# danpovey/quantization

Measured on AMD Instinct MI355X. Metric: vectors encoded/sec at dim=512, 8 codebooks; uint8 codes bit-exact vs ref, higher is better.
Workload: dtype f32 (products: exact 30-bit fixed point on the i8 MFMA); 1 GPU; Quantizer.encode, dim=512, bytes_per_frame=8, codebook_size=256, refine_indexes_iters=5, batch=65536 fp32 Gaussian vectors per GPU (BASELINE.json configs[1]), seeded synthetic codebooks; global_batch=65536, parallelism=batch-sharded x1, no collective

## Files before the change

quantization_amd/csrc/mcq_api.hip:

```cpp
#include "../../include/mcq.h"
#include "mcq_kernels.h"
#include "mcq_fix_kernels.h"
#include "mcq_loss_kernels.h"
#include "mcq_tf_kernels.h"
#include "mcq_pass16_kernels.h"
#include "mcq_train_kernels.h"
#include "mcq_search_kernels.h"
#include "mcq_range_kernels.h"

#include <cstdlib>
#include <type_traits>
#include <utility>
#include <vector>

using namespace mcq;

namespace {

inline int round_up16(int d) { return (d + 15) & ~15; }
inline size_t align256(size_t v) { return (v + 255) & ~size_t(255); }
inline bool is_pow2(int v) { return v > 0 && (v & (v - 1)) == 0; }

int k_cutoff(int K, int L) {
    int kc = (K <= 16) ? 8 : 16;
    while (L >= 4) { L /= 4; kc *= 2; }
    return kc < 128 ? kc : 128;
}

struct Prepared {
    const float *C, *Q, *bias, *scales, *G, *mean, *wmu;
    const int8_t *Cf, *Wf;
    const int *Ce, *We;
};

struct PreparedLayout {
    size_t offC, offQ, offCf, offCe, offWf, offWe, offWmu, offBias, offScales, offMean, offCMean, offG, total;
};

PreparedLayout prepared_layout(int N, int K, int D) {
    const size_t nk = (size_t)N * K, Dp = round_up16(D);
    const size_t planes = fix_plane_bytes((long)nk, D), exps = (size_t)fix_round_rows((long)nk) * 4;
    PreparedLayout l;
    l.offC = 0;
    l.offQ = align256(l.offC + nk * Dp * 4);
    l.offCf = align256(l.offQ + nk * 4);
    l.offCe = align256(l.offCf + planes);
    l.offWf = align256(l.offCe + exps);
    l.offWe = align256(l.offWf + planes);
    l.offWmu = align256(l.offWe + exps);
    l.offBias = align256(l.offWmu + nk * 4);
    l.offScales = align256(l.offBias + nk * 4);
    l.offMean = align256(l.offScales + 8);
    l.offCMean = align256(l.offMean + Dp * 4);
    l.offG = align256(l.offCMean + (size_t)N * Dp * 4);
    l.total = align256(l.offG + nk * nk * 4);
    static_assert(kFixTile == 128, "");
    if (l.total < l.offBias + (nk + kFixTile) * 4) l.total = align256(l.offBias + (nk + kFixTile) * 4);
    return l;
}

Prepared prepared_view(const void *p, int N, int K, int D) {
    const PreparedLayout l = prepared_layout(N, K, D);
    const char *b = static_cast<const char *>(p);
    return Prepared{reinterpret_cast<const float *>(b + l.offC), reinterpret_cast<const float *>(b + l.offQ),
                    reinterpret_cast<const float *>(b + l.offBias), reinterpret_cast<const float *>(b + l.offScales),
                    reinterpret_cast<const float *>(b + l.offG), reinterpret_cast<const float *>(b + l.offMean),
                    reinterpret_cast<const float *>(b + l.offWmu),
                    reinterpret_cast<const int8_t *>(b + l.offCf), reinterpret_cast<const int8_t *>(b + l.offWf),
                    reinterpret_cast<const int *>(b + l.offCe), reinterpret_cast<const int *>(b + l.offWe)};
}

template <typename CT>
struct WorkspaceT {
    CT *idx, *idxB, *idxC, *final_idx;
    int *map[2], *cnt;
    float *E, *R, *xx, *XC;
    float *gterms;
    int8_t *xf;
    int *xe;
    float *tabs[2];
    TfLists tf;
};

int tf_levels(int N) { int v = 0; while ((1 << v) < N) ++v; return v; }

size_t tf_tab_floats(int N, int K) {
    const int nlev = tf_levels(N);
    size_t best = 0;
    for (int v = 2; v < nlev; ++v) {
        const size_t groups = (size_t)N >> (v + 1);
        for (int u = 1; u < v; ++u) {
            const size_t per = (size_t)1 << (v - u), kc = k_cutoff(K, 1 << u);
            const size_t f = groups * per * per * kc * kc;
            best = f > best ? f : best;
        }
    }
    return best;
}

inline size_t code_bytes_of(int K) { return K > 256 ? 2 : 1; }

size_t workspace_per_vector(int N, int K, int D) {
    const size_t cb = code_bytes_of(K);
    return 4 * cb * (size_t)N + 8 + 8 + 4 * (size_t)N + 4 * (size_t)N * K + (size_t)tf_levels(N) * N * (16 * cb + 2 * 16 + 4 * 16) + 64 +
           2 * 4 * tf_tab_floats(N, K) + 4 * (size_t)fix_round_cols(D) + 4 + 4 * (size_t)N * N;
}
size_t workspace_slack(int D) { return 48 * 256 + (size_t)kFixTile * (4 * (size_t)fix_round_cols(D) + 4); }

long default_chunk(int N, int K, int D) {
    long c = (long)(((size_t)2 << 30) / workspace_per_vector(N, K, D));
    c = c > 65536 ? 65536 : c;
    c = c < 1024 ? 1024 : c;
    return c & ~127L;
}

template <typename CT>
WorkspaceT<CT> carve(void *ws, long Bc, int N, int K, int D) {
    char *p = static_cast<char *>(ws);
    size_t off = 0;
    auto take = [&](size_t bytes) { char *q = p + off; off = align256(off + bytes); return q; };
    WorkspaceT<CT> w;
    w.idx = reinterpret_cast<CT *>(take((size_t)Bc * N * sizeof(CT)));
    w.idxB = reinterpret_cast<CT *>(take((size_t)Bc * N * sizeof(CT)));
    w.idxC = reinterpret_cast<CT *>(take((size_t)Bc * N * sizeof(CT)));
    w.final_idx = reinterpret_cast<CT *>(take((size_t)Bc * N * sizeof(CT)));
    for (int i = 0; i < 2; ++i) w.map[i] = reinterpret_cast<int *>(take((size_t)Bc * 4));
    w.cnt = reinterpret_cast<int *>(take(64 * 4));
    w.E = reinterpret_cast<float *>(take((size_t)Bc * 4));
    w.R = reinterpret_cast<float *>(take((size_t)Bc * N * 4));
    w.xx = reinterpret_cast<float *>(take((size_t)Bc * 4));
    w.gterms = reinterpret_cast<float *>(take((size_t)Bc * N * N * 4));
    w.XC = reinterpret_cast<float *>(take((size_t)Bc * N * K * 4));
    w.xf = reinterpret_cast<int8_t *>(take(fix_plane_bytes(Bc, D)));
    w.xe = reinterpret_cast<int *>(take((size_t)fix_round_rows(Bc) * 4));
    const int nlev = tf_levels(N);
    w.tf.ent = nullptr;
    w.tf.out_i64 = nullptr;
    w.tf.out_u8 = nullptr;
    w.tf.out_pack = 1;
    w.tf.map = nullptr;
    w.tf.erG = w.tf.erXC = w.tf.erxx = nullptr;
    w.tf.erE = w.tf.erR = nullptr;
    w.tf.erK = 0;
    for (int v = 0; v < kTfLevels; ++v) {
        w.tf.kc[v] = k_cutoff(K, 1 << v);
        w.tf.pos[v] = nullptr;
        w.tf.S[v] = nullptr;
        if (v >= nlev) continue;
        const int kc = w.tf.kc[v];
        if (v == 0) w.tf.ent = reinterpret_cast<uint8_t *>(take((size_t)Bc * N * kc * sizeof(CT)));
        else w.tf.pos[v] = reinterpret_cast<uint8_t *>(take((size_t)Bc * (N >> v) * kc * 2));
        w.tf.S[v] = reinterpret_cast<float *>(take((size_t)Bc * (N >> v) * kc * 4));
    }
    const size_t tf = tf_tab_floats(N, K);
    for (int i = 0; i < 2; ++i) w.tabs[i] = tf ? reinterpret_cast<float *>(take((size_t)Bc * tf * 4)) : nullptr;
    return w;
}

bool domain_ok(int N, int K, int D) {
    return is_pow2(K) && K >= 16 && K <= 1024 && is_pow2(N) && N <= 64 && (long)N * K <= 16384 && D >= 1 && D <= 16384;
}
int domain_err(int N, int K, int D = 1) {
    return (K < 16 || K > 1024 || N > 64 || (long)N * K > 16384 || D > 16384) ? MCQ_EUNSUPPORTED : MCQ_EINVAL;
}

struct Prof {
    hipStream_t stream;
    int only = -1;
    std::vector<hipEvent_t> ev;
    std::vector<int> cat, first, last;
    int open = -1;
    void begin(int category) {
        if (only >= 0 && category != only) { open = -1; return; }
        if (ev.empty() || open != (int)ev.size() - 1) {
            hipEvent_t e;
            (void)hipEventCreate(&e);
            (void)hipEventRecord(e, stream);
            ev.push_back(e);
        }
        open = (int)ev.size() - 1;
    }
    void untimed() { open = -1; }
    void end(int category) {
        if (only >= 0 && category != only) { open = -1; return; }
        hipEvent_t e;
        (void)hipEventCreate(&e);
        (void)hipEventRecord(e, stream);
        ev.push_back(e);
        first.push_back(open);
        last.push_back((int)ev.size() - 1);
        cat.push_back(category);
        open = (int)ev.size() - 1;
    }
};

thread_local int g_last_launches = 0;

#define MCQ_LAUNCH_CHECK()                               \
    do {                                                 \
        hipError_t e_ = hipGetLastError();               \
        if (e_ != hipSuccess) return (int)e_;            \
        ++g_last_launches;                               \
    } while (0)

FixRowsArgs fix_rows_args(const float *src, int xh, long R, int D, long ld, int8_t *planes, int *exps, float *xx,
                          const float *bias_src = nullptr, float *bias_dst = nullptr, const float *sub = nullptr,
                          long sub_per = 0, long sub_ld = 0, const float *dot_vec = nullptr, float *dot_out = nullptr) {
    return FixRowsArgs{src, xh, R, fix_round_rows(R), D, ld, fix_round_cols(D), planes, exps, xx, bias_src, bias_dst,
                       sub, sub_per, sub_ld, dot_vec, dot_out, nullptr};
}

int launch_fix_rows(const float *src, int xh, long R, int D, long ld, int8_t *planes, int *exps, float *xx, hipStream_t st,
                    const float *sub = nullptr, unsigned *clear = nullptr) {
    FixRowsArgs a = fix_rows_args(src, xh, R, D, ld, planes, exps, xx, nullptr, nullptr, sub, 0, 0);
    a.clear = clear;
    hipLaunchKernelGGL(k_fix_rows<4>, dim3((unsigned)(a.Rp / 4)), dim3(256), 0, st, a);
    MCQ_LAUNCH_CHECK();
    return 0;
}

int launch_fix_rows2(const FixRowsArgs &a, const FixRowsArgs &b, hipStream_t st) {
    const unsigned na = (unsigned)(a.Rp / 4), nb = (unsigned)(b.Rp / 4);
    hipLaunchKernelGGL(k_fix_rows2<4>, dim3(na + nb), dim3(256), 0, st, a, b, na);
    MCQ_LAUNCH_CHECK();
    return 0;
}

template <int MODE>
int launch_fgemm(FixGemm g, hipStream_t st) {
    static bool allowed[64] = {};
    constexpr int lds = MODE == FG_SCREEN ? kFixLdsScreen : kFixLds;
    int dev = 0;
    if (hipGetDevice(&dev) != hipSuccess || dev < 0 || dev >= 64) dev = 63;
    if (!allowed[dev] || dev == 63) {
        const hipError_t attr = hipFuncSetAttribute(reinterpret_cast<const void *>(&k_fgemm<MODE>),
                                                    hipFuncAttributeMaxDynamicSharedMemorySize, lds);
        if (attr != hipSuccess) return (int)attr;
        allowed[dev] = true;
    }
    const long MT = g.RA / kFixTile, NT = g.RB / kFixTile;
    const int H = (MODE != FG_STORE && g.K > kFixTile) ? g.K / kFixTile : 1;
    const long big = g.walk_rows ? NT : MT, small_units = (g.walk_rows ? MT : NT) / H;
    long units = (big + 7) / 8 * small_units;
    if (units > 32) units = 32;
    hipLaunchKernelGGL((k_fgemm<MODE>), dim3((unsigned)(8 * units)), dim3(512), lds, st, g);
    MCQ_LAUNCH_CHECK();
    return 0;
}

int launch_xc(const int8_t *xf, const int *xe, long B, const int8_t *Cf, const int *Ce, long nk, int D, float *out,
              hipStream_t st) {
    FixGemm g{};
    g.A = xf; g.ea = xe; g.RA = fix_round_rows(B); g.M = B;
    g.B = Cf; g.eb = Ce; g.RB = fix_round_rows(nk); g.N = nk;
    g.Dq = fix_round_cols(D);
    g.walk_rows = 0;
    g.out = out; g.ldo = nk;
    return launch_fgemm<FG_STORE>(g, st);
}

inline bool exact_logits_forced() {
    static const bool on = getenv("MCQ_EXACT_LOGITS") && atoi(getenv("MCQ_EXACT_LOGITS")) != 0;
    return on;
}

int launch_logits(const int8_t *xf, const int *xe, long B, const Prepared &P, int N, int K, int D, float lscale,
                  const float *lscale_ptr, float *logits, void *idx, hipStream_t st, unsigned *und_cnt = nullptr,
                  unsigned *und_list = nullptr) {
    const long nk = (long)N * K;
    FixGemm g{};
    g.A = P.Wf; g.ea = P.We; g.RA = fix_round_rows(nk); g.M = nk;
    g.B = xf; g.eb = xe; g.RB = fix_round_rows(B); g.N = B;
    g.Dq = fix_round_cols(D);
    g.walk_rows = 1;
    g.bias = P.bias; g.wmu = P.wmu; g.lscale = lscale; g.lscale_ptr = lscale_ptr;
    g.logits = logits; g.ldo = nk; g.idx = idx; g.idx_wide = K > 256 ? 1 : 0; g.K = K; g.ncb = N;
    if (und_cnt == nullptr) return launch_fgemm<FG_LOGITS>(g, st);
    if (logits != nullptr) return MCQ_EINVAL;
    g.und_cnt = und_cnt; g.und_list = und_list; g.und_cap = (unsigned)(B * N);
    const int rc = launch_fgemm<FG_SCREEN>(g, st);
    if (rc) return rc;
    FixRecheck r{};
    r.W = P.Wf; r.X = xf; r.ew = P.We; r.ex = xe; r.RW = g.RA; r.RX = g.RB; r.Dq = g.Dq;
    r.bias = P.bias; r.wmu = P.wmu; r.lscale_ptr = lscale_ptr; r.lscale = lscale;
    r.idx = idx; r.idx_wide = g.idx_wide; r.K = K; r.ncb = N; r.cnt = und_cnt; r.list = und_list; r.cap = g.und_cap;
    const long waves = B * N;
    hipLaunchKernelGGL(k_fscreen_recheck, dim3((unsigned)(waves < 4096 ? (waves + 3) / 4 : 1024)), dim3(256), 0, st, r);
    MCQ_LAUNCH_CHECK();
    return 0;
}

constexpr unsigned kCapStage0 = 32768, kCapWave = 65536;
inline unsigned pass_grid(unsigned full, bool capped, unsigned cap) { return (capped && full > cap) ? cap : full; }

template <int K>
int launch_tf_stage0_k(int N, const float *G, const float *XC, const tf_code_of<K> *idx, const float *R, const float *Q, long B,
                       int keep, tf_code_of<K> *ent, float *S, tf_code_of<K> *fin, const int *nact, const int *map, hipStream_t st,
                       bool capped) {
    const unsigned vgrid = (unsigned)(((B + 3) / 4) * N);
    const dim3 grid(pass_grid(vgrid, capped, kCapStage0)), block(256);
#define MCQ_S0_CASE(NN)                                                                                                            \
    case NN:                                                                                                                       \
        if (capped) hipLaunchKernelGGL((k_tf_stage0<K, NN, true>), grid, block, 0, st, G, XC, idx, R, Q, B, keep, ent, S, fin, nact, map, vgrid); \
        else hipLaunchKernelGGL((k_tf_stage0<K, NN, false>), grid, block, 0, st, G, XC, idx, R, Q, B, keep, ent, S, fin, nact, map, vgrid);      \
        break;
    switch (N) {
        MCQ_S0_CASE(1) MCQ_S0_CASE(2) MCQ_S0_CASE(4) MCQ_S0_CASE(8) MCQ_S0_CASE(16) MCQ_S0_CASE(32) MCQ_S0_CASE(64)
        default: return MCQ_EUNSUPPORTED;
    }
#undef MCQ_S0_CASE
    MCQ_LAUNCH_CHECK();
    return 0;
}

int launch_tf_stage0(int K, int N, const float *G, const float *XC, const uint16_t *idx, const float *R, const float *Q,
                     long B, int keep, uint16_t *ent, float *S, uint16_t *fin, const int *nact, const int *map, hipStream_t st,
                     bool capped) {
    switch (K) {
        case 512: return launch_tf_stage0_k<512>(N, G, XC, idx, R, Q, B, keep, ent, S, fin, nact, map, st, capped);
        case 1024: return launch_tf_stage0_k<1024>(N, G, XC, idx, R, Q, B, keep, ent, S, fin, nact, map, st, capped);
        default: return MCQ_EUNSUPPORTED;
    }
}

int launch_tf_stage0(int K, int N, const float *G, const float *XC, const uint8_t *idx, const float *R, const float *Q,
                     long B, int keep, uint8_t *ent, float *S, uint8_t *fin, const int *nact, const int *map, hipStream_t st,
                     bool capped) {
    if (K == 16 && N >= 4 && keep <= 16) {
        const dim3 grid((unsigned)((B * (N / 4) + 3) / 4)), block(256);
#define MCQ_S16_CASE(NN) \
    case NN: hipLaunchKernelGGL((k_tf_stage0_k16<NN>), grid, block, 0, st, G, XC, idx, R, Q, B, keep, ent, S, nact, map); break;
        switch (N) {
            MCQ_S16_CASE(4) MCQ_S16_CASE(8) MCQ_S16_CASE(16) MCQ_S16_CASE(32) MCQ_S16_CASE(64)
            default: return MCQ_EUNSUPPORTED;
        }
#undef MCQ_S16_CASE
        MCQ_LAUNCH_CHECK();
        return 0;
    }
    switch (K) {
        case 16: return launch_tf_stage0_k<16>(N, G, XC, idx, R, Q, B, keep, ent, S, fin, nact, map, st, capped);
        case 32: return launch_tf_stage0_k<32>(N, G, XC, idx, R, Q, B, keep, ent, S, fin, nact, map, st, capped);
        case 64: return launch_tf_stage0_k<64>(N, G, XC, idx, R, Q, B, keep, ent, S, fin, nact, map, st, capped);
        case 128: return launch_tf_stage0_k<128>(N, G, XC, idx, R, Q, B, keep, ent, S, fin, nact, map, st, capped);
        case 256: return launch_tf_stage0_k<256>(N, G, XC, idx, R, Q, B, keep, ent, S, fin, nact, map, st, capped);
        default: return MCQ_EUNSUPPORTED;
    }
}

template <typename CT>
int launch_tf_er(int N, const float *G, const float *XC, const CT *idx, const float *xx, long B, int K, float *E, float *R,
                 float *gterms, const int *nact, const int *map, hipStream_t st) {
    const dim3 grid((unsigned)((B + 3) / 4)), block(256);
    const bool direct = B <= 8192;
#define MCQ_ER_CASE(NN)                                                                                                  \
    case NN:                                                                                                             \
        if (!direct) {                                                                                                   \
            hipLaunchKernelGGL((k_tf_gram_terms<NN, CT>), dim3((unsigned)(((B + 4 * (64 / NN) - 1) / (4 * (64 / NN))) * NN)), block, 0, st, G, idx, \
                               B, K, gterms, nact);                                                                      \
            MCQ_LAUNCH_CHECK();                                                                                          \
        }                                                                                                                \
        hipLaunchKernelGGL((k_tf_er<NN, CT>), grid, block, 0, st, gterms, XC, idx, xx, B, K, E, R, nact, map,              \
                           direct ? G : static_cast<const float *>(nullptr));                                           \
        break;
    switch (N) {
        MCQ_ER_CASE(1) MCQ_ER_CASE(2) MCQ_ER_CASE(4) MCQ_ER_CASE(8) MCQ_ER_CASE(16) MCQ_ER_CASE(32) MCQ_ER_CASE(64)
        default: return MCQ_EUNSUPPORTED;
    }
#undef MCQ_ER_CASE
    MCQ_LAUNCH_CHECK();
    return 0;
}

int launch_tf_up(int kh, int kc, const TfLists &L, long B, int N, int u, int ntab, int per, const float *in, float *out,
                 const int *nact, hipStream_t st) {
    const dim3 grid((unsigned)(B * ntab)), block(64);
#define MCQ_UP_CASE(A, C) \
    if (kh == A && kc == C) { hipLaunchKernelGGL((k_tf_up<A, C>), grid, block, 0, st, L, B, N, u, ntab, per, in, out, nact); MCQ_LAUNCH_CHECK(); return 0; }
    MCQ_UP_CASE(16, 32) MCQ_UP_CASE(32, 32) MCQ_UP_CASE(32, 64) MCQ_UP_CASE(8, 16) MCQ_UP_CASE(16, 16)
#undef MCQ_UP_CASE
    return MCQ_EUNSUPPORTED;
}

template <typename CT>
int launch_tf_comb(int kh, int kc, const float *E, const TfLists &L, long B, int N, int v, int keep, const float *tabs,
                   CT *fin, const int *nact, hipStream_t st, bool capped) {
    if (fin == nullptr) capped = false;
    const dim3 grid(pass_grid((unsigned)(B * (N >> (v + 1))), capped, kCapWave)), block(64);
#define MCQ_COMB_CASE(A, C)                                                                                                        \
    if (kh == A && kc == C) {                                                                                                     \
        if (fin && capped) hipLaunchKernelGGL((k_tf_comb<A, C, true, CT, true>), grid, block, 0, st, E, L, B, N, v, keep, tabs, fin, nact); \
        else if (fin) hipLaunchKernelGGL((k_tf_comb<A, C, true, CT>), grid, block, 0, st, E, L, B, N, v, keep, tabs, fin, nact);  \
        else hipLaunchKernelGGL((k_tf_comb<A, C, false, CT>), grid, block, 0, st, E, L, B, N, v, keep, tabs, fin, nact);          \
        MCQ_LAUNCH_CHECK();                                                                                                       \
        return 0;                                                                                                                 \
    }
    MCQ_COMB_CASE(16, 32) MCQ_COMB_CASE(32, 32) MCQ_COMB_CASE(32, 64) MCQ_COMB_CASE(64, 64)
    if constexpr (sizeof(CT) == 1) { MCQ_COMB_CASE(8, 16) MCQ_COMB_CASE(16, 16) }
#undef MCQ_COMB_CASE
    return MCQ_EUNSUPPORTED;
}

enum { CAT_LOGITS = 0, CAT_XX = 1, CAT_STAGE0 = 2, CAT_XC = 3, CAT_LEVEL0 = 4, CAT_LEVEL1 = 5, CAT_TABLES = 6, CAT_COMBINE = 7,
       CAT_TABLES_UP = 8, CAT_COMBINE_UP = 9, CAT_ER = 10, CAT_LEVEL1_FUSED = 11, CAT_TAIL = 12, CAT_COUNT = 13 };
const char *const kCatNames[CAT_COUNT] = {
    "logits_product_argmax",
    "frames_to_limbs",
    "stage0_tables",
    "xc_product",
    "combine_level0",
    "combine_level1",
    "tables_level1",
    "combine_level2",
    "tables_upper_levels",
    "combine_upper_levels",
    "residual_energies",
    "level1_combines_and_tables",
    "encode_tail",
};

#define MCQ_TF_LAUNCH2(SMALLK, BIGK, grid, block, ...)                                                       \
    do {                                                                                                     \
        bool s_ = false;                                                                                     \
        if constexpr (sizeof(CT) == 1) {                                                                     \
            if (small) { hipLaunchKernelGGL(SMALLK, grid, block, 0, st, __VA_ARGS__); s_ = true; }           \
        }                                                                                                    \
        if (!s_) hipLaunchKernelGGL(BIGK, grid, block, 0, st, __VA_ARGS__);                                  \
    } while (0)
inline bool pass16_enabled() {
    static const bool on = !(getenv("MCQ_PASS16") && atoi(getenv("MCQ_PASS16")) == 0);
    return on;
}
inline long skip_min_batch() {
    const char *v = getenv("MCQ_SKIP_MIN_BATCH");
    return v ? atol(v) : 8192;
}

template <typename CT>
int run_tf_combines(const float *G, const CT *idx_cur, CT *idx_new, const WorkspaceT<CT> &w, const TfLists &L, long B, int N,
                    int K, const int *nact, hipStream_t st, Prof *prof, bool capped) {
    const bool small = (K == 16);
    const int nlev = tf_levels(N);
    {
        const int keep = (N == 2) ? 1 : L.kc[1];
        CT *fin = (N == 2) ? idx_new : nullptr;
        const dim3 grid((unsigned)(B * (N / 2)));
        if (prof) prof->begin(CAT_LEVEL0);
        bool done0 = false;
        if constexpr (sizeof(CT) == 1) {
            if (!small) {
                if (capped)
                    hipLaunchKernelGGL(k_tf_pair0s<true>, dim3(pass_grid(grid.x, true, kCapWave)), dim3(64), 0, st, G, idx_cur, w.E, L, B, N,
                                       K, keep, fin, nact);
                else
                    hipLaunchKernelGGL(k_tf_pair0s<false>, grid, dim3(64), 0, st, G, idx_cur, w.E, L, B, N, K, keep, fin, nact);
                done0 = true;
            }
        }
        if (!done0) MCQ_TF_LAUNCH2((k_tf_pair0<8, CT>), (k_tf_pair0<16, CT>), grid, dim3(64), G, idx_cur, w.E, L, B, N, K, keep, fin, nact);
        MCQ_LAUNCH_CHECK();
        if (prof) prof->end(CAT_LEVEL0);
    }
    const bool fuse_l1 = (N >= 8);
    const bool fuse_l3 = fuse_l1 && N == 16 && small;
    if (fuse_l1) {
        const int keep = L.kc[2];
        const int groups2 = N >> 3, per1 = 2, ntab1 = groups2 * per1 * per1;
        const unsigned pair_blocks = (unsigned)(B * (N / 4)), tab_blocks = (unsigned)(B * ntab1);
        const int ntab3 = fuse_l3 ? 16 : 1, per3 = fuse_l3 ? 4 : 1;
        const unsigned vgrid = pair_blocks + tab_blocks + (fuse_l3 ? (unsigned)(B * ntab3) : 0u);
        const dim3 grid(pass_grid(vgrid, capped, kCapWave));
        if (prof) prof->begin(CAT_LEVEL1_FUSED);
        if (capped)
            MCQ_TF_LAUNCH2((k_tf_level1<8, 8, CT, true>), (k_tf_level1<16, 16, CT, true>), grid, dim3(64), G, idx_cur, w.E, L, B, N, K, keep, ntab1,
                           per1, w.tabs[0], nact, pair_blocks, tab_blocks, ntab3, per3, w.tabs[1], vgrid);
        else
            MCQ_TF_LAUNCH2((k_tf_level1<8, 8, CT>), (k_tf_level1<16, 16, CT>), grid, dim3(64), G, idx_cur, w.E, L, B, N, K, keep, ntab1, per1, w.tabs[0],
                           nact, pair_blocks, tab_blocks, ntab3, per3, w.tabs[1], vgrid);
        MCQ_LAUNCH_CHECK();
        if (prof) prof->end(CAT_LEVEL1_FUSED);
    } else if (N >= 4) {
        const int keep = (N == 4) ? 1 : L.kc[2];
        CT *fin = (N == 4) ? idx_new : nullptr;
        const dim3 grid((unsigned)(B * (N / 4)));
        if (prof) prof->begin(CAT_LEVEL1);
        MCQ_TF_LAUNCH2((k_tf_pair1<8, 8, CT>), (k_tf_pair1<16, 16, CT>), grid, dim3(64), G, idx_cur, w.E, L, B, N, K, keep, fin, nact);
        MCQ_LAUNCH_CHECK();
        if (prof) prof->end(CAT_LEVEL1);
    }
    for (int v = 2; v < nlev; ++v) {
        const int groups = N >> (v + 1);
        const bool last = (v == nlev - 1);
        const int keep = last ? 1 : L.kc[v + 1];
        CT *fin = last ? idx_new : nullptr;
        const int per1 = 1 << (v - 1), ntab1 = groups * per1 * per1;
        const int cat_tab = (v == 2) ? CAT_TABLES : CAT_TABLES_UP, cat_comb = (v == 2) ? CAT_COMBINE : CAT_COMBINE_UP;
        if (!(fuse_l1 && v == 2) && !(fuse_l3 && v == 3)) {
            if (prof) prof->begin(cat_tab);
            MCQ_TF_LAUNCH2((k_tf_table1<8, 8, CT>), (k_tf_table1<16, 16, CT>), dim3((unsigned)(B * ntab1)), dim3(64), G, idx_cur, L, B, N, K, ntab1, per1,
                           w.tabs[0], nact);
            MCQ_LAUNCH_CHECK();
            if (prof) prof->end(cat_tab);
        }
        if (N == 16 && v == 3) {
            if (prof) prof->begin(cat_comb);
            const float *t3 = fuse_l3 ? w.tabs[1] : w.tabs[0];
            MCQ_TF_LAUNCH2((k_tf_comb3<8, 16, 16, CT>), (k_tf_comb3<16, 32, 32, CT>), dim3((unsigned)B), dim3(256), idx_cur, w.E, L, B, N, t3, idx_new, nact);
            MCQ_LAUNCH_CHECK();
            if (prof) prof->end(cat_comb);
            continue;
        }
        int cur = 0;
        for (int u = 2; u < v; ++u) {
            const int per = 1 << (v - u), ntab = groups * per * per;
            if (prof) prof->begin(cat_tab);
            const int rc = launch_tf_up(L.kc[u - 1], L.kc[u], L, B, N, u, ntab, per, w.tabs[cur], w.tabs[cur ^ 1], nact, st);
            if (rc) return rc;
            if (prof) prof->end(cat_tab);
            cur ^= 1;
        }
        if (prof) prof->begin(cat_comb);
        const int rc = launch_tf_comb<CT>(L.kc[v - 1], L.kc[v], w.E, L, B, N, v, keep, w.tabs[cur], fin, nact, st, capped);
        if (rc) return rc;
        if (prof) prof->end(cat_comb);
    }
    return 0;
}
#undef MCQ_TF_LAUNCH2

template <typename CT>
int run_encode_t(const float *x, long B, const void *prepared, float lscale, int N, int K, int D, int iters,
                 uint8_t *out_u8, int64_t *out_i64, void *workspace, size_t workspace_bytes, hipStream_t st,
                 Prof *prof, const int64_t *init_idx, unsigned flags, float *logits_out,
                 uint8_t *codes_also ) {
    g_last_launches = 0;
    if (!domain_ok(N, K, D)) return domain_err(N, K, D);
    if (B < 0 || iters < 0 || iters > 60 || (out_u8 == nullptr) == (out_i64 == nullptr)) return MCQ_EINVAL;
    if (sizeof(CT) > 1 && (out_u8 != nullptr || codes_also != nullptr)) return MCQ_EINVAL;
    if (B == 0) return 0;
    if (!x || !prepared || !workspace) return MCQ_EINVAL;
    const size_t per = workspace_per_vector(N, K, D), slack = workspace_slack(D);
    if (workspace_bytes < slack + per) return MCQ_EWORKSPACE;
    long chunk = (long)((workspace_bytes - slack) / per);
    if (chunk > B) chunk = B;
    if (chunk < B && chunk < 128) return MCQ_EWORKSPACE;
    if (chunk < B) chunk &= ~127L;
    const Prepared P = prepared_view(prepared, N, K, D);
    const int pack = (out_u8 != nullptr && K == 16 && N >= 2) ? 2 : 1;
    const bool want_skip = (flags & MCQ_ENCODE_ALL_PASSES) == 0 && iters >= 3;

    for (long lo = 0; lo < B; lo += chunk) {
        const long Bc = (B - lo < chunk) ? (B - lo) : chunk;
        const WorkspaceT<CT> w = carve<CT>(workspace, Bc, N, K, D);
        const int xh = (flags & MCQ_ENCODE_X_FP16) ? 1 : 0;
        const float *xc = xh ? reinterpret_cast<const float *>(reinterpret_cast<const uint16_t *>(x) + lo * D) : x + lo * D;
        int rc;
        const bool screen = init_idx == nullptr && logits_out == nullptr && (flags & MCQ_ENCODE_EXACT_LOGITS) == 0 &&
                            !exact_logits_forced() && (size_t)Bc * N < ((size_t)1 << 31);
        unsigned *const und_cnt = reinterpret_cast<unsigned *>(w.cnt + 63), *const und_list = reinterpret_cast<unsigned *>(w.XC);
        if (init_idx == nullptr || iters > 0) {
            if (prof) prof->begin(CAT_XX);
            rc = launch_fix_rows(xc, xh, Bc, D, D, w.xf, w.xe, w.xx, st, P.mean, screen ? und_cnt : nullptr);
            if (rc) return rc;
            if (prof) prof->end(CAT_XX);
        }
        if (init_idx != nullptr) {
            hipLaunchKernelGGL(k_import_indexes<CT>, dim3((unsigned)((Bc * N + 255) / 256)), dim3(256), 0, st,
                               init_idx + lo * N, Bc * N, K, w.idx);
            MCQ_LAUNCH_CHECK();
            if (prof) prof->untimed();
        } else {
            if (prof) prof->begin(CAT_LOGITS);
            rc = launch_logits(w.xf, w.xe, Bc, P, N, K, D, lscale,
                               (flags & MCQ_ENCODE_LSCALE_FROM_PREPARED) ? P.scales + 1 : nullptr,
                               logits_out ? logits_out + lo * N * K : nullptr, w.idx, st, screen ? und_cnt : nullptr, und_list);
            if (rc) return rc;
            if (prof) prof->end(CAT_LOGITS);
        }
        if (iters > 0) {
            if (prof) prof->begin(CAT_XC);
            rc = launch_xc(w.xf, w.xe, Bc, P.Cf, P.Ce, (long)N * K, D, w.XC, st);
            if (rc) return rc;
            if (prof) prof->end(CAT_XC);
        }
        const bool use_p16 = sizeof(CT) == 1 && K == 16 && (N == 16 || N == 8) && iters > 0 && prof == nullptr && pass16_enabled();
        const bool skip = want_skip && !use_p16 && Bc >= skip_min_batch();
        int iters_left = iters;
        CT *idx_cur = w.idx, *idx_new = skip ? w.idxB : w.idx, *idx_pk = w.idxC;
        const int *map_cur = nullptr, *nact = nullptr;
        int *map_nxt = w.map[0], *map_spare = w.map[1];
        float *E_cur = w.E, *R_cur = w.R, *E_alt = w.gterms, *R_alt = w.gterms + ((Bc + 3) & ~3L);
        if (skip) {
            hipLaunchKernelGGL(k_zero_counts, dim3(1), dim3(64), 0, st, w.cnt, 64);
            MCQ_LAUNCH_CHECK();
            if (prof) prof->untimed();
        }
        bool wrote_direct = false;
        if constexpr (sizeof(CT) == 1) {
            if (use_p16) {
                static bool allowed16[64] = {};
                int dev = 0;
                if (hipGetDevice(&dev) != hipSuccess || dev < 0 || dev >= 64) dev = 63;
                if (!allowed16[dev] || dev == 63) {
                    hipError_t attr = hipFuncSetAttribute(reinterpret_cast<const void *>(&k_tf_pass16<16>),
                                                          hipFuncAttributeMaxDynamicSharedMemorySize, p16_lds_bytes<16>());
                    if (attr == hipSuccess)
                        attr = hipFuncSetAttribute(reinterpret_cast<const void *>(&k_tf_pass16<8>),
                                                   hipFuncAttributeMaxDynamicSharedMemorySize, p16_lds_bytes<8>());
                    if (attr != hipSuccess) return (int)attr;
                    allowed16[dev] = true;
                }
                Pass16Args a;
                a.G = P.G; a.XC = w.XC; a.xx = w.xx; a.Q = P.Q; a.idx = w.idx; a.B = Bc; a.iters = iters;
                const bool direct_out = pack == 1;
                a.out_i64 = (direct_out && out_i64) ? out_i64 + lo * N : nullptr;
                a.out_u8 = direct_out ? (out_u8 ? out_u8 + lo * N : (codes_also ? codes_also + lo * N : nullptr)) : nullptr;
                const long wgs = (Bc + kP16Waves - 1) / kP16Waves;
                if (N == 16)
                    hipLaunchKernelGGL(k_tf_pass16<16>, dim3((unsigned)(wgs < 256 ? wgs : 256)), dim3(64 * kP16Waves), p16_lds_bytes<16>(), st, a);
                else
                    hipLaunchKernelGGL(k_tf_pass16<8>, dim3((unsigned)(wgs < 512 ? wgs : 512)), dim3(64 * kP16Waves), p16_lds_bytes<8>(), st, a);
                MCQ_LAUNCH_CHECK();
                if (direct_out) continue;
                iters_left = 0;
            }
        }
        const bool er_in_emit = (N == 4 || N == 8 || N == 16);
        bool er_ready = false;
        for (int it = 0; it < iters_left; ++it) {
            const bool last_pass = (it + 1 == iters);
            const bool capped = skip && it >= 3;
            if (!er_ready) {
                if (prof) prof->begin(CAT_ER);
                rc = launch_tf_er<CT>(N, P.G, w.XC, idx_cur, w.xx, Bc, K, E_cur, R_cur, w.gterms, nact, map_cur, st);
                if (rc) return rc;
                if (prof) prof->end(CAT_ER);
            }
            er_ready = false;
            if (prof) prof->begin(CAT_STAGE0);
            rc = launch_tf_stage0(K, N, P.G, w.XC, idx_cur, R_cur, P.Q, Bc, (N == 1) ? 1 : w.tf.kc[0], reinterpret_cast<CT *>(w.tf.ent),
                                  w.tf.S[0], (N == 1) ? idx_new : static_cast<CT *>(nullptr), nact, map_cur, st, capped);
            if (rc) return rc;
            if (prof) prof->end(CAT_STAGE0);
            bool direct_out = false;
            if (N >= 2) {
                TfLists L = w.tf;
                L.map = map_cur;
                if (er_in_emit && !last_pass) {
                    L.erG = P.G; L.erXC = w.XC; L.erxx = w.xx; L.erE = E_cur; L.erR = R_cur; L.erK = K;
                    er_ready = true;
                }
                direct_out = last_pass;
                if (direct_out) {
                    L.out_i64 = out_i64 ? out_i64 + lo * N : nullptr;
                    L.out_u8 = out_u8 ? out_u8 + lo * (N / pack) : (codes_also ? codes_also + lo * N : nullptr);
                    L.out_pack = out_u8 ? pack : 1;
                    wrote_direct = true;
                }
                WorkspaceT<CT> wc = w;
                wc.E = E_cur;
                wc.R = R_cur;
                rc = run_tf_combines<CT>(P.G, idx_cur, idx_new, wc, L, Bc, N, K, nact, st, prof, capped);
                if (rc) return rc;
            }
            if (skip && !direct_out) {
                if (prof) prof->begin(CAT_TAIL);
                hipLaunchKernelGGL(k_compact<CT>, dim3((unsigned)((Bc + 255) / 256)), dim3(256), 0, st, idx_cur, idx_new,
                                   map_cur, nact, Bc, N, last_pass ? 1 : 0, idx_pk, map_nxt, w.cnt + it,
                                   er_ready ? E_cur : nullptr, er_ready ? R_cur : nullptr, E_alt, R_alt, pack,
                                   out_u8 ? out_u8 + lo * (N / pack) : nullptr, out_i64 ? out_i64 + lo * N : nullptr,
                                   codes_also ? codes_also + lo * N : nullptr);
                MCQ_LAUNCH_CHECK();
                if (prof) prof->end(CAT_TAIL);
                CT *t = idx_cur; idx_cur = idx_pk; idx_pk = t;
                int *old_map = const_cast<int *>(map_cur);
                map_cur = map_nxt;
                map_nxt = old_map ? old_map : map_spare;
                nact = w.cnt + it;
                if (er_ready) {
                    std::swap(E_cur, E_alt);
                    std::swap(R_cur, R_alt);
                }
            }
        }
        if (wrote_direct || skip) continue;
        const long outn = (out_i64 != nullptr) ? Bc * N : Bc * (N / pack);
        if (prof) prof->begin(CAT_TAIL);
        hipLaunchKernelGGL(k_finalize<CT>, dim3((unsigned)((outn + 255) / 256)), dim3(256), 0, st, w.idx, Bc, N, pack,
                           out_u8 ? out_u8 + lo * (N / pack) : nullptr, out_i64 ? out_i64 + lo * N : nullptr,
                           codes_also ? codes_also + lo * N : nullptr);
        MCQ_LAUNCH_CHECK();
        if (prof) prof->end(CAT_TAIL);
    }
    return 0;
}

int run_encode(const float *x, long B, const void *prepared, float lscale, int N, int K, int D, int iters,
               uint8_t *out_u8, int64_t *out_i64, void *workspace, size_t workspace_bytes, hipStream_t st,
               Prof *prof, const int64_t *init_idx = nullptr, unsigned flags = 0, float *logits_out = nullptr,
               uint8_t *codes_also = nullptr) {
    if (K > 256)
        return run_encode_t<uint16_t>(x, B, prepared, lscale, N, K, D, iters, out_u8, out_i64, workspace, workspace_bytes, st, prof,
                                      init_idx, flags, logits_out, codes_also);
    return run_encode_t<uint8_t>(x, B, prepared, lscale, N, K, D, iters, out_u8, out_i64, workspace, workspace_bytes, st, prof,
                                 init_idx, flags, logits_out, codes_also);
}

int db_cw_of(int D, int K) {
    if ((D & 3) != 0) return 1;
    if (K >= 64) return 4;
    return D >= 1024 ? 4 : (D >= 512 ? 2 : 1);
}
int db_cw(const void *g, const void *out, int D, int K, long gsb, long gsn, const void *dotw = nullptr) {
    const bool al = ((D & 3) == 0) && ((gsb & 3) == 0) && ((gsn & 3) == 0) && ((reinterpret_cast<uintptr_t>(g) & 15) == 0) &&
                    ((reinterpret_cast<uintptr_t>(out) & 15) == 0) && ((reinterpret_cast<uintptr_t>(dotw) & 15) == 0);
    return al ? db_cw_of(D, K) : 1;
}
int db_chunks(int D, int cw) { return (D + 64 * cw - 1) / (64 * cw); }

template <typename IdxT>
int launch_decode_backward(const float *g, const IdxT *idx, long B, int N, int K, int D, float *out, long gsb, long gsn,
                           int idx_stride, hipStream_t st, const float *sa = nullptr, const float *sb = nullptr, float sc = 1.0f,
                           const float *dotw = nullptr, float *dot_part = nullptr) {
    const int cw = db_cw(g, out, D, K, gsb, gsn, dotw), chunks = db_chunks(D, cw);
    const long rowgroups = ((long)N * K + 3) / 4;
    long blocks;
    if (chunks <= 8 && (8 % chunks) == 0) blocks = ((rowgroups + (8 / chunks) - 1) / (8 / chunks)) * 8;
    else blocks = ((long)N * K * chunks + 3) / 4;
    const dim3 grid((unsigned)blocks), block(256);
    if (cw == 4) hipLaunchKernelGGL((k_decode_backward<IdxT, 4>), grid, block, 0, st, g, idx, B, N, K, D, chunks, out, gsb, gsn, idx_stride, sa, sb, sc, dotw, dot_part);
    else if (cw == 2) hipLaunchKernelGGL((k_decode_backward<IdxT, 2>), grid, block, 0, st, g, idx, B, N, K, D, chunks, out, gsb, gsn, idx_stride, sa, sb, sc, dotw, dot_part);
    else hipLaunchKernelGGL((k_decode_backward<IdxT, 1>), grid, block, 0, st, g, idx, B, N, K, D, chunks, out, gsb, gsn, idx_stride, sa, sb, sc, dotw, dot_part);
    hipError_t e = hipGetLastError();
    return e == hipSuccess ? 0 : (int)e;
}
}

namespace {

int search_domain(int N, int K, int D) {
    if (!domain_ok(N, K, D)) return domain_err(N, K, D);
    return K > 256 ? MCQ_EUNSUPPORTED : 0;
}

int search_check(const float *tables, long Q, const uint8_t *codes, const float *w, long B, int N, int K, int k, int metric,
                 bool outs_ok, const void *workspace) {
    if (const int rc = search_domain(N, K, 1)) return rc;
    if (k > 64) return MCQ_EUNSUPPORTED;
    if (k < 1 || Q < 0 || B < 0 || Q > 0x7fffffffL) return MCQ_EINVAL;
    if (metric != MCQ_SEARCH_L2 && metric != MCQ_SEARCH_IP && metric != MCQ_SEARCH_COS) return MCQ_EINVAL;
    if (B > 0x7fffffffL) return MCQ_EUNSUPPORTED;
    if (!outs_ok) return MCQ_EINVAL;
    if (Q == 0 || B == 0) return 0;
    if (!tables || !codes || !workspace) return MCQ_EINVAL;
    if (!w && metric != MCQ_SEARCH_IP) return MCQ_EINVAL;
    const int need = N >= 16 ? 16 : N;
    if (reinterpret_cast<uintptr_t>(codes) % need != 0) return MCQ_EINVAL;
    return 0;
}

inline int launch_rc() {
    const hipError_t e = hipGetLastError();
    return e == hipSuccess ? 0 : (int)e;
}

int allow_dynamic_lds(bool (&allowed)[64], const void *kernel, int bytes) {
    int dev = 0;
    if (hipGetDevice(&dev) != hipSuccess || dev < 0 || dev >= 64) dev = 63;
    if (!allowed[dev] || dev == 63) {
        const hipError_t attr = hipFuncSetAttribute(kernel, hipFuncAttributeMaxDynamicSharedMemorySize, bytes);
        if (attr != hipSuccess) return (int)attr;
        allowed[dev] = true;
    }
    return 0;
}

template <bool RNORM>
int code_norms(const uint8_t *codes, long B, const void *prepared, int N, int K, int D, float *out, void *stream) {
    if (const int rc = search_domain(N, K, D)) return rc;
    if (B < 0) return MCQ_EINVAL;
    if (B > 0x7fffffffL) return MCQ_EUNSUPPORTED;
    if (B == 0) return 0;
    if (!codes || !prepared || !out) return MCQ_EINVAL;
    const Prepared P = prepared_view(prepared, N, K, D);
    hipLaunchKernelGGL(k_code_norms<RNORM>, dim3((unsigned)((B + kNormWaves - 1) / kNormWaves)), dim3(64 * kNormWaves), 0,
                       static_cast<hipStream_t>(stream), codes, B, P.C, N, K, round_up16(D), out);
    return launch_rc();
}

struct TilePlan {
    int qt, qtiles, slices;
    long per_slice;
};

TilePlan tile_plan(long Q, long B, int N, int K, int waves) {
    TilePlan p;
    int cap = kScanQTMax;
    while (cap > 1 && (size_t)cap * N * K * 4 > (size_t)kScanTableLds) cap /= 2;
    int qt = 1;
    while (qt < cap && qt < Q) qt *= 2;
    p.qt = qt;
    p.qtiles = (int)((Q + qt - 1) / qt);
    long cap_slices = kScanTargetBlocks / (p.qtiles > 0 ? p.qtiles : 1);
    cap_slices = cap_slices < 1 ? 1 : (cap_slices > kScanMaxSlices ? kScanMaxSlices : cap_slices);
    const long steps = (B + 63) / 64;
    long want = (steps + waves - 1) / waves;
    want = want < 1 ? 1 : (want > cap_slices ? cap_slices : want);
    p.per_slice = (((B + want - 1) / want) + 63) / 64 * 64;
    if (p.per_slice < 64) p.per_slice = 64;
    p.slices = (int)((B + p.per_slice - 1) / p.per_slice);
    return p;
}

struct ScanPlan : TilePlan {
    size_t lds, ws_half;
};

ScanPlan scan_plan(long Q, long B, int N, int K, int k) {
    ScanPlan p{tile_plan(Q, B, N, K, kScanWaves), 0, 0};
    const size_t tab = (size_t)p.qt * N * K * 4, lists = (size_t)p.qt * kScanWaves * 64 * 8;
    p.lds = tab > lists ? tab : lists;
    p.ws_half = align256((size_t)Q * p.slices * k * 4);
    return p;
}

template <int QT, int NN, int M>
int launch_scan(const ScanPlan &p, hipStream_t st, const float *tables, int Q, const uint8_t *codes, const float *norms, long B,
                int K, int k, float *ws_s, int *ws_i) {
    static bool allowed[64] = {};
    if (const int rc = allow_dynamic_lds(allowed, reinterpret_cast<const void *>(&k_search_scan<QT, NN, M>), kScanTableLds))
        return rc;
    hipLaunchKernelGGL((k_search_scan<QT, NN, M>), dim3((unsigned)p.qtiles * (unsigned)p.slices), dim3(64 * kScanWaves), p.lds, st,
                       tables, Q, codes, norms, B, K, k, p.slices, p.per_slice, ws_s, ws_i);
    return launch_rc();
}

template <int QT, int M>
int launch_scan_n(const ScanPlan &p, hipStream_t st, const float *tables, int Q, const uint8_t *codes, const float *norms,
                  long B, int N, int K, int k, float *ws_s, int *ws_i) {
    switch (N) {
#define MCQ_SCAN_CASE(NN) \
    case NN: return launch_scan<QT, NN, M>(p, st, tables, Q, codes, norms, B, K, k, ws_s, ws_i);
        MCQ_SCAN_CASE(1) MCQ_SCAN_CASE(2) MCQ_SCAN_CASE(4) MCQ_SCAN_CASE(8) MCQ_SCAN_CASE(16) MCQ_SCAN_CASE(32) MCQ_SCAN_CASE(64)
#undef MCQ_SCAN_CASE
    }
    return MCQ_EUNSUPPORTED;
}

static_assert(kMetricL2 == MCQ_SEARCH_L2 && kMetricIP == MCQ_SEARCH_IP && kMetricCos == MCQ_SEARCH_COS, "include/mcq.h");
template <int M>
int launch_scan_qt(const ScanPlan &p, hipStream_t st, const float *tables, int Q, const uint8_t *codes, const float *w, long B,
                   int N, int K, int k, float *ws_s, int *ws_i) {
    switch (p.qt) {
        case 1: return launch_scan_n<1, M>(p, st, tables, Q, codes, w, B, N, K, k, ws_s, ws_i);
        case 2: return launch_scan_n<2, M>(p, st, tables, Q, codes, w, B, N, K, k, ws_s, ws_i);
        case 4: return launch_scan_n<4, M>(p, st, tables, Q, codes, w, B, N, K, k, ws_s, ws_i);
        case 8: return launch_scan_n<8, M>(p, st, tables, Q, codes, w, B, N, K, k, ws_s, ws_i);
        case 16: return launch_scan_n<16, M>(p, st, tables, Q, codes, w, B, N, K, k, ws_s, ws_i);
    }
    return MCQ_EUNSUPPORTED;
}

}


namespace {

struct RangePlan : TilePlan {
    size_t lds, ws_bytes;
};

RangePlan range_plan(long Q, long B, int N, int K) {
    RangePlan p{tile_plan(Q, B, N, K, kRangeWaves), 0, 0};
    p.lds = (size_t)p.qt * N * K * 4 + (size_t)kRangeWaves * p.qt * 8;
    p.ws_bytes = align256((size_t)Q * p.slices * kRangeWaves * 8);
    return p;
}

struct RangeArgs {
    const float *tables;
    int Q;
    const uint8_t *codes;
    const float *w;
    long B;
    int N, K, metric;
    const float *thr;
    int64_t *ws;
    const int64_t *lims;
    float *out_s;
    int64_t *out_i;
    long capacity;
};

template <int QT, int CH, bool FILL>
int launch_range(const RangePlan &p, hipStream_t st, const RangeArgs &a) {
    static bool allowed[64] = {};
    if (const int rc = allow_dynamic_lds(allowed, reinterpret_cast<const void *>(&k_range_sweep<QT, CH, FILL>),
                                         kScanTableLds + kRangeWaves * kScanQTMax * 8))
        return rc;
    hipLaunchKernelGGL((k_range_sweep<QT, CH, FILL>), dim3((unsigned)p.qtiles * (unsigned)p.slices), dim3(64 * kRangeWaves), p.lds,
                       st, a.tables, a.Q, a.codes, a.w, a.B, a.N, a.K, a.metric, p.slices, p.per_slice, a.thr, a.ws, a.lims,
                       a.out_s, a.out_i, a.capacity);
    return launch_rc();
}

template <int QT, bool FILL>
int launch_range_ch(const RangePlan &p, hipStream_t st, const RangeArgs &a) {
    switch (a.N < 8 ? a.N : 8) {
        case 1: return launch_range<QT, 1, FILL>(p, st, a);
        case 2: return launch_range<QT, 2, FILL>(p, st, a);
        case 4: return launch_range<QT, 4, FILL>(p, st, a);
        case 8: return launch_range<QT, 8, FILL>(p, st, a);
    }
    return MCQ_EUNSUPPORTED;
}

template <bool FILL>
int launch_range_qt(const RangePlan &p, hipStream_t st, const RangeArgs &a) {
    switch (p.qt) {
        case 1: return launch_range_ch<1, FILL>(p, st, a);
        case 2: return launch_range_ch<2, FILL>(p, st, a);
        case 4: return launch_range_ch<4, FILL>(p, st, a);
        case 8: return launch_range_ch<8, FILL>(p, st, a);
        case 16: return launch_range_ch<16, FILL>(p, st, a);
    }
    return MCQ_EUNSUPPORTED;
}

int range_check(const float *tables, long Q, const uint8_t *codes, const float *w, long B, int N, int K, int metric,
                const float *thr, const int64_t *lims, const void *workspace, size_t workspace_bytes) {
    if (const int rc = search_check(tables, Q, codes, w, B, N, K, 1, metric, lims != nullptr, workspace)) return rc;
    if (Q == 0 || B == 0) return 0;
    if (!thr) return MCQ_EINVAL;
    if (workspace_bytes < range_plan(Q, B, N, K).ws_bytes) return MCQ_EWORKSPACE;
    return 0;
}

}


extern "C" {

int mcq_abi_version(void) { return MCQ_ABI_VERSION; }

int mcq_padded_dim(int D) { return round_up16(D); }

size_t mcq_prepared_bytes(int N, int K, int D) {
    if (N <= 0 || K <= 0 || D <= 0) return 0;
    return prepared_layout(N, K, D).total;
}

static int prepare_impl(const float *centers, float cscale_exp, const float *scales_dev, const float *weight,
                        const float *bias, int N, int K, int D, void *prepared, void *stream, const float *raw_cs = nullptr,
                        const float *raw_ls = nullptr, float speed = 0.f, float *scales_out2 = nullptr) {
    if (!domain_ok(N, K, D)) return domain_err(N, K, D);
    if (!centers || !prepared || ((weight == nullptr) != (bias == nullptr))) return MCQ_EINVAL;
    hipStream_t st = static_cast<hipStream_t>(stream);
    const PreparedLayout l = prepared_layout(N, K, D);
    char *b = static_cast<char *>(prepared);
    const long rows = (long)N * K;
    const int Dp = round_up16(D);
    const unsigned grid = (unsigned)((rows + 3) / 4);
    hipLaunchKernelGGL(k_prepare_rows, dim3(grid), dim3(256), 0, st, centers, cscale_exp, 1, rows, D, Dp,
                       reinterpret_cast<float *>(b + l.offC), static_cast<float *>(nullptr) , scales_dev,
                       (scales_dev || raw_cs) ? reinterpret_cast<float *>(b + l.offScales) : static_cast<float *>(nullptr), raw_cs,
                       raw_ls, speed, scales_out2);
    hipError_t e = hipGetLastError();
    if (e != hipSuccess) return (int)e;
    if (!weight) return 0;
    const float *C = reinterpret_cast<const float *>(b + l.offC);
    float *cmean = reinterpret_cast<float *>(b + l.offCMean);
    hipLaunchKernelGGL(k_centers_mean, dim3((unsigned)(Dp / 16)), dim3(1024), 0, st, C, N, K, Dp,
                       reinterpret_cast<float *>(b + l.offMean), cmean);
    e = hipGetLastError();
    if (e != hipSuccess) return (int)e;
    int rc = launch_fix_rows2(fix_rows_args(C, 0, rows, Dp, Dp, reinterpret_cast<int8_t *>(b + l.offCf), reinterpret_cast<int *>(b + l.offCe),
                                            reinterpret_cast<float *>(b + l.offQ), nullptr, nullptr, cmean, K, Dp),
                              fix_rows_args(weight, 0, rows, D, D, reinterpret_cast<int8_t *>(b + l.offWf), reinterpret_cast<int *>(b + l.offWe),
                                            nullptr, bias, reinterpret_cast<float *>(b + l.offBias), nullptr, 0, 0,
                                            reinterpret_cast<const float *>(b + l.offMean), reinterpret_cast<float *>(b + l.offWmu)), st);
    if (rc) return rc;
    {
        rc = launch_xc(reinterpret_cast<const int8_t *>(b + l.offCf), reinterpret_cast<const int *>(b + l.offCe), rows,
                       reinterpret_cast<const int8_t *>(b + l.offCf), reinterpret_cast<const int *>(b + l.offCe), rows, D,
                       reinterpret_cast<float *>(b + l.offG), st);
        if (rc) return rc;
    }
    return 0;
}

size_t mcq_prepared_decode_bytes(int N, int K, int D) {
    if (N <= 0 || K <= 0 || D <= 0) return 0;
    return prepared_layout(N, K, D).offCf;
}

size_t mcq_prepared_mean_offset(int N, int K, int D) {
    if (N <= 0 || K <= 0 || D <= 0) return 0;
    return prepared_layout(N, K, D).offMean;
}

int mcq_prepare(const float *centers, float cscale_exp, const float *weight, const float *bias, int N, int K, int D,
                void *prepared, void *stream) {
    return prepare_impl(centers, cscale_exp, nullptr, weight, bias, N, K, D, prepared, stream);
}

int mcq_prepare_dev(const float *centers, const float *scales_exp, const float *weight, const float *bias, int N,
                    int K, int D, void *prepared, void *stream) {
    if (!scales_exp) return MCQ_EINVAL;
    return prepare_impl(centers, 1.0f, scales_exp, weight, bias, N, K, D, prepared, stream);
}

int mcq_prepare_params(const float *centers, const float *centers_scale, const float *logits_scale, float speed,
                       const float *weight, const float *bias, int N, int K, int D, void *prepared, float *scales_exp_out,
                       void *stream) {
    if (!centers_scale || !logits_scale) return MCQ_EINVAL;
    return prepare_impl(centers, 1.0f, nullptr, weight, bias, N, K, D, prepared, stream, centers_scale, logits_scale, speed,
                        scales_exp_out);
}

size_t mcq_encode_workspace_bytes(long B, int N, int K, int D) {
    if (B <= 0 || N <= 0 || K <= 0 || D <= 0 || !domain_ok(N, K, D)) return 48 * 256;
    const long dc = default_chunk(N, K, D), chunk = B < dc ? B : dc;
    return workspace_slack(D) + workspace_per_vector(N, K, D) * (size_t)chunk;
}

int mcq_encode(const float *x, long B, const void *prepared, float lscale_exp, int N, int K, int D, int refine_iters,
               uint8_t *out_u8, int64_t *out_i64, void *workspace, size_t workspace_bytes, void *stream) {
    return run_encode(x, B, prepared, lscale_exp, N, K, D, refine_iters, out_u8, out_i64, workspace,
                      workspace_bytes, static_cast<hipStream_t>(stream), nullptr);
}

int mcq_encode_ex(const float *x, long B, const void *prepared, float lscale_exp, int N, int K, int D,
                  int refine_iters, uint8_t *out_u8, int64_t *out_i64, void *workspace, size_t workspace_bytes,
                  void *stream, unsigned flags) {
    return run_encode(x, B, prepared, lscale_exp, N, K, D, refine_iters, out_u8, out_i64, workspace,
                      workspace_bytes, static_cast<hipStream_t>(stream), nullptr, nullptr, flags);
}

int mcq_refine_indexes(const float *x, long B, const void *prepared, int N, int K, int D, int refine_iters,
                       const int64_t *idx_in, int64_t *idx_out, void *workspace, size_t workspace_bytes,
                       void *stream) {
    if (B > 0 && (!idx_in || !idx_out)) return MCQ_EINVAL;
    return run_encode(x, B, prepared, 1.0f, N, K, D, refine_iters, nullptr, idx_out, workspace, workspace_bytes,
                      static_cast<hipStream_t>(stream), nullptr, B > 0 ? idx_in : nullptr);
}

int mcq_decode(const void *codes, int code_bytes, int codes_per_row, long B, const void *prepared, int N, int K, int D,
               float *out, void *stream) {
    if (!domain_ok(N, K, D)) return domain_err(N, K);
    if (B < 0 || codes_per_row <= 0 || N % codes_per_row != 0) return MCQ_EINVAL;
    const int rep = N / codes_per_row;
    if (!(rep == 1 || rep == 2 || rep == 4 || rep == 8 || rep == 16)) return MCQ_EINVAL;
    if (code_bytes != 1 && code_bytes != 8) return MCQ_EINVAL;
    if (B == 0) return 0;
    if (!codes || !prepared || !out) return MCQ_EINVAL;
    hipStream_t st = static_cast<hipStream_t>(stream);
    const Prepared P = prepared_view(prepared, N, K, D);
    const int Dp = round_up16(D);
    const unsigned grid = (unsigned)((B + 3) / 4);
    const int J = (Dp / 4 + 63) / 64;
    static const bool sliced_ok = !(getenv("MCQ_DECODE_SLICED") && atoi(getenv("MCQ_DECODE_SLICED")) == 0);
    const char *lds_env = getenv("MCQ_DECODE_LDS_MIN");
    const long lds_min_b = lds_env ? atol(lds_env) : 16384;
    {
        const char *blk_env = getenv("MCQ_DECODE_BLK");
        const int blk_mode = blk_env ? atoi(blk_env) : 1;
        const size_t lds_max = 160 * 1024, cbytes = 2 * 16384;
        int lpv = 0;
        if ((size_t)N * K * 64 + cbytes <= lds_max) lpv = 4;
        else if ((size_t)N * K * 32 + cbytes <= lds_max) lpv = 2;
        if (blk_mode != 0 && sliced_ok && rep == 1 && code_bytes == 1 && B >= lds_min_b && K >= 32 && (D & 3) == 0 && lpv != 0 &&
            (N == 4 || N == 8 || N == 16) && ((reinterpret_cast<uintptr_t>(codes) & 15) == 0) && ((reinterpret_cast<uintptr_t>(out) & 15) == 0)) {
            const int W = 4 * lpv, ns = Dp / W, per_xcd = (ns + 7) / 8;
            int groups = 256 / (8 * per_xcd);
            groups = groups < 1 ? 1 : groups;
            const unsigned g = (unsigned)(8 * per_xcd * groups);
            const long per = (((B + groups - 1) / groups) + 255) / 256 * 256;
            const size_t lds = (size_t)N * K * W * 4 + cbytes;
            const uint8_t *cp = static_cast<const uint8_t *>(codes);
#define MCQ_DECB(NN, LL)                                                                                                    \
    do {                                                                                                                    \
        static bool allowed[64] = {};                                                                                       \
        int dev = 0;                                                                                                        \
        if (hipGetDevice(&dev) != hipSuccess || dev < 0 || dev >= 64) dev = 63;                                             \
        if (!allowed[dev] || dev == 63) {                                                                                   \
            const hipError_t attr = hipFuncSetAttribute(reinterpret_cast<const void *>(&k_decode_blk<NN, LL>),              \
                                                        hipFuncAttributeMaxDynamicSharedMemorySize, (int)lds_max);          \
            if (attr != hipSuccess) return (int)attr;                                                                       \
            allowed[dev] = true;                                                                                            \
        }                                                                                                                   \
        hipLaunchKernelGGL((k_decode_blk<NN, LL>), dim3(g), dim3(1024), lds, st, cp, B, P.C, K, D, Dp, groups, per, out);   \
    } while (0)
            if (N == 4) { if (lpv == 4) MCQ_DECB(4, 4); else MCQ_DECB(4, 2); }
            else if (N == 8) { if (lpv == 4) MCQ_DECB(8, 4); else MCQ_DECB(8, 2); }
            else { if (lpv == 4) MCQ_DECB(16, 4); else MCQ_DECB(16, 2); }
#undef MCQ_DECB
            hipError_t e6 = hipGetLastError();
            return e6 == hipSuccess ? 0 : (int)e6;
        }
    }
    if (sliced_ok && rep == 1 && B >= lds_min_b && (size_t)N * K * 64 <= 144 * 1024 && K >= 32 && N >= 8) {
        const int ns = Dp / 16, per_xcd = (ns + 7) / 8;
        int groups = 256 / (8 * per_xcd);
        groups = groups < 1 ? 1 : groups;
        const unsigned g = (unsigned)(8 * per_xcd * groups);
        const size_t lds = (size_t)N * K * 64;
        if (code_bytes == 1)
            hipLaunchKernelGGL((k_decode_lds<uint8_t>), dim3(g), dim3(1024), lds, st, static_cast<const uint8_t *>(codes), B,
                               P.C, N, K, D, Dp, groups, out);
        else
            hipLaunchKernelGGL((k_decode_lds<int64_t>), dim3(g), dim3(1024), lds, st, static_cast<const int64_t *>(codes), B,
                               P.C, N, K, D, Dp, groups, out);
        hipError_t e4 = hipGetLastError();
        return e4 == hipSuccess ? 0 : (int)e4;
    }
    if (sliced_ok && rep == 1 && B >= 4096 && K >= 32) {
        int lpv = 4;
        while (lpv * 32 < Dp) lpv *= 2;
        if (lpv <= 64) {
            const int vpw = 64 / lpv;
            const unsigned g = (unsigned)(((B + 4 * vpw - 1) / (4 * vpw)) * 8);
#define MCQ_DECS_LAUNCH(T, CHH, LL)                                                                              \
    hipLaunchKernelGGL((k_decode_sliced<T, CHH, LL>), dim3(g), dim3(256), 0, st, static_cast<const T *>(codes), B, P.C, N, \
                       K, D, Dp, out)
#define MCQ_DECS_LPV(T, CHH)                                                                                     \
    switch (lpv) {                                                                                               \
        case 4: MCQ_DECS_LAUNCH(T, CHH, 4); break;                                                               \
        case 8: MCQ_DECS_LAUNCH(T, CHH, 8); break;                                                               \
        case 16: MCQ_DECS_LAUNCH(T, CHH, 16); break;                                                             \
        case 32: MCQ_DECS_LAUNCH(T, CHH, 32); break;                                                             \
        default: MCQ_DECS_LAUNCH(T, CHH, 64); break;                                                             \
    }
            if (code_bytes == 1) {
                if (N <= 4) { MCQ_DECS_LPV(uint8_t, 4) } else if (N <= 8) { MCQ_DECS_LPV(uint8_t, 8) } else { MCQ_DECS_LPV(uint8_t, 16) }
            } else {
                if (N <= 4) { MCQ_DECS_LPV(int64_t, 4) } else if (N <= 8) { MCQ_DECS_LPV(int64_t, 8) } else { MCQ_DECS_LPV(int64_t, 16) }
            }
#undef MCQ_DECS_LPV
#undef MCQ_DECS_LAUNCH
            hipError_t e3 = hipGetLastError();
            return e3 == hipSuccess ? 0 : (int)e3;
        }
    }
#define MCQ_DEC_CASE(NN, JJ)                                                                                    \
    if (code_bytes == 1 && rep == 1 && N == NN && J == JJ) {                                                    \
        hipLaunchKernelGGL((k_decode_reg<NN, JJ>), dim3(grid), dim3(256), 0, st, static_cast<const uint8_t *>(codes), \
                           B, P.C, K, D, Dp, out);                                                              \
        hipError_t e2 = hipGetLastError();                                                                      \
        return e2 == hipSuccess ? 0 : (int)e2;                                                                  \
    }
    MCQ_DEC_CASE(8, 2)
    MCQ_DEC_CASE(8, 1)
    MCQ_DEC_CASE(4, 1)
    MCQ_DEC_CASE(4, 2)
    MCQ_DEC_CASE(4, 4)
    MCQ_DEC_CASE(16, 1)
    MCQ_DEC_CASE(16, 2)
    MCQ_DEC_CASE(2, 1)
    MCQ_DEC_CASE(2, 2)
#undef MCQ_DEC_CASE
    if (code_bytes == 1)
        hipLaunchKernelGGL((k_decode<uint8_t>), dim3(grid), dim3(256), 0, st, static_cast<const uint8_t *>(codes),
                           codes_per_row, B, P.C, N, K, D, Dp, out);
    else
        hipLaunchKernelGGL((k_decode<int64_t>), dim3(grid), dim3(256), 0, st, static_cast<const int64_t *>(codes),
                           codes_per_row, B, P.C, N, K, D, Dp, out);
    hipError_t e = hipGetLastError();
    return e == hipSuccess ? 0 : (int)e;
}

int mcq_decode_backward(const float *grad_out, const int64_t *idx, long B, int N, int K, int D, float *gC,
                        void *stream) {
    if (N <= 0 || K <= 0 || D <= 0 || B < 0 || !gC) return MCQ_EINVAL;
    if (B > 0 && (!grad_out || !idx)) return MCQ_EINVAL;
    return launch_decode_backward<int64_t>(grad_out, idx, B, N, K, D, gC, (long)D, 0L, N, static_cast<hipStream_t>(stream));
}

int mcq_decode_backward_u8(const float *grad_out, const uint8_t *codes, long B, int N, int K, int D, float *gC,
                           void *stream) {
    if (K > 256) return MCQ_EUNSUPPORTED;
    if (N <= 0 || K <= 0 || D <= 0 || B < 0 || !gC) return MCQ_EINVAL;
    if (B > 0 && (!grad_out || !codes)) return MCQ_EINVAL;
    return launch_decode_backward<uint8_t>(grad_out, codes, B, N, K, D, gC, (long)D, 0L, N, static_cast<hipStream_t>(stream));
}

int mcq_scatter_rows(const float *grad, long stride_b, long stride_n, const int64_t *idx, int idx_stride, long B, int N,
                     int K, int D, float *out, void *stream) {
    if (N <= 0 || K <= 0 || D <= 0 || B < 0 || !out || idx_stride < N) return MCQ_EINVAL;
    if (B > 0 && (!grad || !idx)) return MCQ_EINVAL;
    return launch_decode_backward<int64_t>(grad, idx, B, N, K, D, out, stride_b, stride_n, idx_stride, static_cast<hipStream_t>(stream));
}

int mcq_jcl_prefix_fwd(const float *hp, const float *emb, const int64_t *idx, long B, int N, int K, int H, float scale,
                       float *A, void *stream) {
    if (N < 2 || K < 1 || H < 1 || B < 0) return MCQ_EINVAL;
    if (B == 0) return 0;
    if (!hp || !emb || !idx || !A) return MCQ_EINVAL;
    hipLaunchKernelGGL(k_jcl_prefix_fwd, dim3((unsigned)((B + 3) / 4)), dim3(256), 0, static_cast<hipStream_t>(stream), hp,
                       emb, idx, B, N, K, H, scale, A);
    hipError_t e = hipGetLastError();
    return e == hipSuccess ? 0 : (int)e;
}

int mcq_jcl_prefix_bwd(const float *A, const float *gA, long B, int N, int H, float scale, float *g_hp, float *gE,
                       void *stream) {
    if (N < 2 || H < 1 || B < 0) return MCQ_EINVAL;
    if (B == 0) return 0;
    if (!A || !gA || !g_hp || !gE) return MCQ_EINVAL;
    hipLaunchKernelGGL(k_jcl_prefix_bwd, dim3((unsigned)((B + 3) / 4)), dim3(256), 0, static_cast<hipStream_t>(stream), A,
                       gA, B, N, H, scale, g_hp, gE);
    hipError_t e = hipGetLastError();
    return e == hipSuccess ? 0 : (int)e;
}

namespace {
struct LogitsWs {
    uint8_t *idx8;
    int8_t *xf;
    int *xe;
    size_t total;
};
LogitsWs logits_ws(void *ws, long B, int N, int D) {
    char *p = static_cast<char *>(ws);
    LogitsWs w;
    size_t off = 0;
    w.idx8 = reinterpret_cast<uint8_t *>(p + off);
    off = align256(off + (size_t)B * N);
    w.xf = reinterpret_cast<int8_t *>(p + off);
    off = align256(off + fix_plane_bytes(B, D));
    w.xe = reinterpret_cast<int *>(p + off);
    off = align256(off + (size_t)fix_round_rows(B) * 4);
    w.total = off;
    return w;
}
}

size_t mcq_logits_workspace_bytes(long B, int N, int D) {
    if (B <= 0 || N <= 0 || D <= 0) return 256;
    return logits_ws(nullptr, B, N, D).total;
}

int mcq_logits(const float *x, long B, const void *prepared, float lscale_exp, int N, int K, int D, float *out,
               void *workspace, size_t workspace_bytes, void *stream) {
    if (!domain_ok(N, K, D)) return MCQ_EUNSUPPORTED;
    if (B == 0) return 0;
    if (!x || !prepared || !out || B < 0 || !workspace) return MCQ_EINVAL;
    if (workspace_bytes < mcq_logits_workspace_bytes(B, N, D)) return MCQ_EWORKSPACE;
    hipStream_t st = static_cast<hipStream_t>(stream);
    const Prepared P = prepared_view(prepared, N, K, D);
    const LogitsWs w = logits_ws(workspace, B, N, D);
    int rc = launch_fix_rows(x, 0, B, D, D, w.xf, w.xe, nullptr, st, P.mean);
    if (rc) return rc;
    return launch_logits(w.xf, w.xe, B, P, N, K, D, lscale_exp, nullptr, out, nullptr, st);
}

int mcq_logits_argmax(const float *x, long B, const void *prepared, float lscale_exp, int N, int K, int D,
                      float *logits_out, int64_t *argmax_out, void *workspace, size_t workspace_bytes, void *stream,
                      unsigned flags) {
    if (!domain_ok(N, K, D) || K > 256) return MCQ_EUNSUPPORTED;
    if (B < 0) return MCQ_EINVAL;
    if (B == 0) return 0;
    if (!x || !prepared || !logits_out || !argmax_out || !workspace) return MCQ_EINVAL;
    if (workspace_bytes < mcq_logits_workspace_bytes(B, N, D)) return MCQ_EWORKSPACE;
    hipStream_t st = static_cast<hipStream_t>(stream);
    const Prepared P = prepared_view(prepared, N, K, D);
    const LogitsWs w = logits_ws(workspace, B, N, D);
    int rc = launch_fix_rows(x, (flags & MCQ_ENCODE_X_FP16) ? 1 : 0, B, D, D, w.xf, w.xe, nullptr, st, P.mean);
    if (rc) return rc;
    rc = launch_logits(w.xf, w.xe, B, P, N, K, D, lscale_exp,
                       (flags & MCQ_ENCODE_LSCALE_FROM_PREPARED) ? P.scales + 1 : nullptr, logits_out, w.idx8, st);
    if (rc) return rc;
    hipLaunchKernelGGL(k_export_indexes, dim3((unsigned)((B * N + 255) / 256)), dim3(256), 0, st, w.idx8, B * N, argmax_out);
    MCQ_LAUNCH_CHECK();
    return 0;
}

int mcq_logits_refine(const float *x, long B, const void *prepared, float lscale_exp, int N, int K, int D, int refine_iters,
                      float *logits_out, int64_t *idx_out, void *workspace, size_t workspace_bytes, void *stream,
                      unsigned flags) {
    return mcq_logits_refine_codes(x, B, prepared, lscale_exp, N, K, D, refine_iters, logits_out, idx_out, nullptr, workspace,
                                   workspace_bytes, stream, flags);
}

int mcq_logits_refine_codes(const float *x, long B, const void *prepared, float lscale_exp, int N, int K, int D, int refine_iters,
                            float *logits_out, int64_t *idx_out, uint8_t *codes_out, void *workspace, size_t workspace_bytes,
                            void *stream, unsigned flags) {
    if (K > 256) return MCQ_EUNSUPPORTED;
    if (B > 0 && (!logits_out || !idx_out)) return MCQ_EINVAL;
    return run_encode(x, B, prepared, lscale_exp, N, K, D, refine_iters, nullptr, idx_out, workspace, workspace_bytes,
                      static_cast<hipStream_t>(stream), nullptr, nullptr, flags | MCQ_ENCODE_ALL_PASSES, logits_out,
                      codes_out);
}

namespace {
long loss_rows_per_chunk(long B) {
    long r = (B + 1023) / 1024;
    r = r < 64 ? 64 : r;
    return (r + 15) / 16 * 16;
}
long loss_chunks(long B) { const long r = loss_rows_per_chunk(B); return (B + r - 1) / r; }
}

size_t mcq_loss_workspace_bytes(long B, int N, int K) {
    if (B <= 0) return 256;
    return (size_t)loss_chunks(B) * N * (2 * (size_t)K + 1) * sizeof(float) + 256;
}

int mcq_loss_fwd(const float *logits, const int64_t *idx, long B, int N, int K, float *lse, float *chosen_sum,
                 float *prob_sum, float *count, void *workspace, size_t workspace_bytes, void *stream) {
    if (!is_pow2(K) || K < 16 || K > 256 || N < 1) return MCQ_EUNSUPPORTED;
    if (B <= 0) return MCQ_EINVAL;
    if (!logits || !idx || !lse || !chosen_sum || !prob_sum || !count || !workspace) return MCQ_EINVAL;
    if (workspace_bytes < mcq_loss_workspace_bytes(B, N, K)) return MCQ_EWORKSPACE;
    hipStream_t st = static_cast<hipStream_t>(stream);
    const long rpc = loss_rows_per_chunk(B), chunks = loss_chunks(B);
    float *pp = static_cast<float *>(workspace);
    float *pc = pp + chunks * N * K;
    float *ph = pc + chunks * N * K;
    const dim3 grid((unsigned)(chunks * N)), block(64 * kLossWaves);
#define MCQ_LOSS_CASE(KK)                                                                                             \
    case KK: hipLaunchKernelGGL((k_loss_fwd<KK>), grid, block, 0, st, logits, idx, B, N, rpc, lse, pp, pc, ph); break;
    switch (K) {
        MCQ_LOSS_CASE(16) MCQ_LOSS_CASE(32) MCQ_LOSS_CASE(64) MCQ_LOSS_CASE(128) MCQ_LOSS_CASE(256)
        default: return MCQ_EUNSUPPORTED;
    }
#undef MCQ_LOSS_CASE
    MCQ_LAUNCH_CHECK();
    hipLaunchKernelGGL(k_loss_reduce, dim3((unsigned)N), dim3(256), 0, st, pp, pc, ph, chunks, N, K, prob_sum, count,
                       chosen_sum);
    MCQ_LAUNCH_CHECK();
    return 0;
}

int mcq_loss_bwd(const float *logits, const int64_t *idx, const float *lse, long B, int N, int K, const float *g_chosen,
                 const float *g_prob, float *grad_logits, void *stream) {
    if (!is_pow2(K) || K < 16 || K > 256 || N < 1) return MCQ_EUNSUPPORTED;
    if (B <= 0) return MCQ_EINVAL;
    if (!logits || !idx || !lse || !g_chosen || !g_prob || !grad_logits) return MCQ_EINVAL;
    hipStream_t st = static_cast<hipStream_t>(stream);
    const int rpw = K < 64 ? 64 / K : 1;
    const long rows = B * N;
    const dim3 grid((unsigned)((rows + (long)kLossWaves * rpw - 1) / ((long)kLossWaves * rpw))), block(64 * kLossWaves);
#define MCQ_LOSS_CASE(KK)                                                                                             \
    case KK: hipLaunchKernelGGL((k_loss_bwd<KK>), grid, block, 0, st, logits, idx, lse, B, N, g_chosen, g_prob, grad_logits); break;
    switch (K) {
        MCQ_LOSS_CASE(16) MCQ_LOSS_CASE(32) MCQ_LOSS_CASE(64) MCQ_LOSS_CASE(128) MCQ_LOSS_CASE(256)
        default: return MCQ_EUNSUPPORTED;
    }
#undef MCQ_LOSS_CASE
    MCQ_LAUNCH_CHECK();
    return 0;
}

int mcq_loss_tail(const float *sums, const float *prob_sum, const float *count, int N, int K, float entropy_scale,
                  float *losses, float *g, float *g_prob, void *stream) {
    if (!is_pow2(K) || K < 16 || K > 256 || N < 1 || N > 64) return MCQ_EUNSUPPORTED;
    if (!sums || !prob_sum || !count || !losses || !g || !g_prob) return MCQ_EINVAL;
    hipLaunchKernelGGL(k_loss_tail, dim3(1), dim3(256), 0, static_cast<hipStream_t>(stream), sums, prob_sum, count, N, K,
                       entropy_scale, losses, g, g_prob);
    MCQ_LAUNCH_CHECK();
    return 0;
}

int mcq_recon_fwd(const float *x, const int64_t *idx, long B, const void *prepared, const float *mean, int N, int K,
                  int D, float *err, float *num_part, float *den_part, void *stream) {
    if (!domain_ok(N, K, D) || K > 256) return MCQ_EUNSUPPORTED;
    if (B <= 0) return MCQ_EINVAL;
    if (!x || !idx || !prepared || !mean || !err || !num_part || !den_part) return MCQ_EINVAL;
    const Prepared P = prepared_view(prepared, N, K, D);
    hipLaunchKernelGGL(k_recon_fwd, dim3((unsigned)((B + 3) / 4)), dim3(256), 0, static_cast<hipStream_t>(stream), x, idx, B,
                       P.C, mean, N, K, D, round_up16(D), err, num_part, den_part);
    MCQ_LAUNCH_CHECK();
    return 0;
}


namespace {
bool wgrad_use_bf3(long B, int M, int D) {
    static const bool f32_only = getenv("MCQ_WGRAD_F32") && atoi(getenv("MCQ_WGRAD_F32")) != 0;
    return !f32_only && (M % kWbM) == 0 && (D % kWbN) == 0 && M >= 1024 && B >= 2048;
}
int wgrad_splits_bf3(long B, int M, int D) {
    const long tiles = (long)(M / kWbM) * (D / kWbN);
    long s = (256 + tiles / 2) / tiles;
    const long max_s = B / 512;
    s = s > max_s ? max_s : s;
    return (int)(s < 1 ? 1 : s);
}

int wgrad_splits(long B, int M, int D) {
    const long tiles = (long)((M + kWgM - 1) / kWgM) * ((D + kWgN - 1) / kWgN);
    long s = 2048 / tiles;
    const long max_s = (B + 127) / 128;
    s = s > max_s ? max_s : s;
    return (int)(s < 1 ? 1 : (s > 64 ? 64 : s));
}
}

size_t mcq_weight_grad_workspace_bytes(long B, int M, int D) {
    if (B <= 0 || M <= 0 || D <= 0) return 256;
    return (size_t)wgrad_splits(B, M, D) * ((size_t)M * D + M) * sizeof(float) + 256;
}

int mcq_weight_grad(const float *G, const float *x, long B, int M, int D, const float *scale_dev, float *gW, float *gb,
                    void *workspace, size_t workspace_bytes, void *stream) {
    if (B <= 0 || M <= 0 || D <= 0 || (M & 15) != 0) return MCQ_EINVAL;
    if (!G || !x || !scale_dev || !gW || !gb || !workspace) return MCQ_EINVAL;
    if (workspace_bytes < mcq_weight_grad_workspace_bytes(B, M, D)) return MCQ_EWORKSPACE;
    hipStream_t st = static_cast<hipStream_t>(stream);
    const bool bf3 = wgrad_use_bf3(B, M, D);
    const int splits = bf3 ? wgrad_splits_bf3(B, M, D) : wgrad_splits(B, M, D);
    long rps = (B + splits - 1) / splits;
    rps = (rps + 31) / 32 * 32;
    float *part = static_cast<float *>(workspace);
    float *partb = part + (size_t)splits * M * D;
    if (bf3) {
        hipLaunchKernelGGL(k_wgrad_bf3, dim3((unsigned)((M / kWbM) * (D / kWbN) * splits)), dim3(512), 0, st, G, x, B, M, D, rps, part, partb);
    } else {
        const unsigned grid = (unsigned)(((M + kWgM - 1) / kWgM) * ((D + kWgN - 1) / kWgN) * splits);
        hipLaunchKernelGGL((k_wgrad_tn<16>), dim3(grid), dim3(256), 0, st, G, x, B, M, D, rps, part, partb);
    }
    MCQ_LAUNCH_CHECK();
    const long MN = (long)M * D;
    hipLaunchKernelGGL(k_wgrad_reduce, dim3((unsigned)((MN / 4 + 255) / 256)), dim3(256), 0, st, part, partb, splits, MN, M,
                       scale_dev, gW, gb);
    MCQ_LAUNCH_CHECK();
    return 0;
}

int mcq_adam_step(float *p, const float *g, float *m, float *v, long n, double lr, double beta1, double beta2, double eps,
                  double weight_decay, double bias_correction1, double bias_correction2_sqrt, void *stream) {
    if (n < 0 || (n > 0 && (!p || !g || !m || !v))) return MCQ_EINVAL;
    if (n == 0) return 0;
    long blocks = (n / 4 + 255) / 256;
    blocks = blocks < 1 ? 1 : (blocks > 2048 ? 2048 : blocks);
    hipLaunchKernelGGL(k_adam, dim3((unsigned)blocks), dim3(256), 0, static_cast<hipStream_t>(stream), p, g, m, v, n,
                       (float)(lr / bias_correction1), (float)(1.0 - beta1), (float)beta2, (float)(1.0 - beta2), (float)eps,
                       (float)weight_decay, (float)bias_correction2_sqrt);
    MCQ_LAUNCH_CHECK();
    return 0;
}

int mcq_loss_head_tail(const float *num_part, const float *den_part, long nparts, const float *chosen_n, int N, float batch,
                       float *head, const float *prob_sum, const float *count, int K, float entropy_scale, float *losses,
                       float *g, float *g_prob, void *stream) {
    if (!is_pow2(K) || K < 16 || K > 256 || N < 1 || N > 64) return MCQ_EUNSUPPORTED;
    if (nparts <= 0 || !num_part || !den_part || !chosen_n || !head || !prob_sum || !count || !losses || !g || !g_prob) return MCQ_EINVAL;
    hipLaunchKernelGGL(k_loss_head_tail, dim3(1), dim3(256), 0, static_cast<hipStream_t>(stream), num_part, den_part, nparts,
                       chosen_n, N, batch, head, prob_sum, count, K, entropy_scale, losses, g, g_prob);
    MCQ_LAUNCH_CHECK();
    return 0;
}
int mcq_loss_head(const float *num_part, const float *den_part, long nparts, const float *chosen_n, int N, float batch,
                  float *head, void *stream) {
    if (nparts <= 0 || N <= 0 || !num_part || !den_part || !chosen_n || !head) return MCQ_EINVAL;
    hipLaunchKernelGGL(k_loss_head, dim3(1), dim3(256), 0, static_cast<hipStream_t>(stream), num_part, den_part, nparts, chosen_n,
                       N, batch, head);
    MCQ_LAUNCH_CHECK();
    return 0;
}

int mcq_scales_exp(const float *centers_scale, const float *logits_scale, float speed, float *out2, void *stream) {
    if (!centers_scale || !logits_scale || !out2) return MCQ_EINVAL;
    hipLaunchKernelGGL(k_scales, dim3(1), dim3(64), 0, static_cast<hipStream_t>(stream), centers_scale, logits_scale, speed, out2);
    MCQ_LAUNCH_CHECK();
    return 0;
}

long mcq_decode_backward_waves(int N, int K, int D) { return (long)N * K * db_chunks(D, db_cw_of(D, K)); }

int mcq_decode_backward_u8_ex(const float *grad_out, const uint8_t *codes, long B, int N, int K, int D, float *gC,
                              const float *sa, const float *sb, float sc, const float *dotw, float *dot_part, void *stream) {
    if (K > 256) return MCQ_EUNSUPPORTED;
    if (N <= 0 || K <= 0 || D <= 0 || B < 0 || !gC) return MCQ_EINVAL;
    if (B > 0 && (!grad_out || !codes)) return MCQ_EINVAL;
    if ((dotw == nullptr) != (dot_part == nullptr)) return MCQ_EINVAL;
    if ((D & 3) == 0 && db_cw(grad_out, gC, D, K, D, 0, dotw) != db_cw_of(D, K)) return MCQ_EINVAL;
    const int rc = launch_decode_backward<uint8_t>(grad_out, codes, B, N, K, D, gC, (long)D, 0L, N, static_cast<hipStream_t>(stream),
                                                   sa, sb, sc, dotw, dot_part);
    if (rc) return rc;
    ++g_last_launches;
    return 0;
}

long mcq_loss_bwd_waves(long B, int N, int K) {
    const int rpw = K < 64 ? 64 / K : 1;
    const long rows = B * N;
    return ((rows + (long)kLossWaves * rpw - 1) / ((long)kLossWaves * rpw)) * kLossWaves;
}

int mcq_loss_bwd_ex(const float *logits, const int64_t *idx, const float *lse, long B, int N, int K, const float *g_chosen,
                    const float *g_prob, float *grad_logits, const float *bias, float *dot_part, void *stream) {
    if (!is_pow2(K) || K < 16 || K > 256 || N < 1) return MCQ_EUNSUPPORTED;
    if (B <= 0) return MCQ_EINVAL;
    if (!logits || !idx || !lse || !g_chosen || !g_prob || !grad_logits || !bias || !dot_part) return MCQ_EINVAL;
    hipStream_t st = static_cast<hipStream_t>(stream);
    const int rpw = K < 64 ? 64 / K : 1;
    const long rows = B * N;
    const dim3 grid((unsigned)((rows + (long)kLossWaves * rpw - 1) / ((long)kLossWaves * rpw))), block(64 * kLossWaves);
#define MCQ_LOSS_CASE(KK)                                                                                             \
    case KK: hipLaunchKernelGGL((k_loss_bwd<KK>), grid, block, 0, st, logits, idx, lse, B, N, g_chosen, g_prob, grad_logits, bias, dot_part); break;
    switch (K) {
        MCQ_LOSS_CASE(16) MCQ_LOSS_CASE(32) MCQ_LOSS_CASE(64) MCQ_LOSS_CASE(128) MCQ_LOSS_CASE(256)
        default: return MCQ_EUNSUPPORTED;
    }
#undef MCQ_LOSS_CASE
    MCQ_LAUNCH_CHECK();
    return 0;
}

int mcq_grad_tail(const float *part_c, long n_c, const float *sa, const float *sb, float sc, const float *part_l, long n_l,
                  float speed, float *out_c, float *out_l, void *stream) {
    if (n_c < 0 || n_l < 0 || (n_c > 0 && !part_c) || (n_l > 0 && !part_l)) return MCQ_EINVAL;
    hipLaunchKernelGGL(k_grad_tail, dim3(1), dim3(1024), 0, static_cast<hipStream_t>(stream), part_c, n_c, sa, sb, sc, part_l, n_l,
                       speed, out_c, out_l);
    MCQ_LAUNCH_CHECK();
    return 0;
}

int mcq_search_tables(const void *q, int q_is_fp16, long Q, const void *prepared, int N, int K, int D, float *tables_out,
                      void *stream) {
    if (const int rc = search_domain(N, K, D)) return rc;
    if (Q < 0 || Q > 0x7fffffffL) return MCQ_EINVAL;
    if (Q == 0) return 0;
    if (!q || !prepared || !tables_out) return MCQ_EINVAL;
    const Prepared P = prepared_view(prepared, N, K, D);
    const int NK = N * K;
    hipLaunchKernelGGL(k_search_tables, dim3((unsigned)((Q + kTabQueries - 1) / kTabQueries), (unsigned)((NK + kTabRows - 1) / kTabRows)),
                       dim3(256), 0, static_cast<hipStream_t>(stream), q, q_is_fp16 ? 1 : 0, (int)Q, P.C, NK, D, round_up16(D),
                       tables_out);
    return launch_rc();
}

int mcq_code_norms(const uint8_t *codes, long B, const void *prepared, int N, int K, int D, float *norms_out, void *stream) {
    return code_norms<false>(codes, B, prepared, N, K, D, norms_out, stream);
}

size_t mcq_search_workspace_bytes(long Q, long B, int N, int K, int k) {
    if (Q <= 0 || B <= 0 || k < 1 || k > 64 || B > 0x7fffffffL || Q > 0x7fffffffL || search_domain(N, K, 1) != 0) return 256;
    return 2 * scan_plan(Q, B, N, K, k).ws_half;
}

int mcq_code_rnorms(const uint8_t *codes, long B, const void *prepared, int N, int K, int D, float *rnorms_out, void *stream) {
    return code_norms<true>(codes, B, prepared, N, K, D, rnorms_out, stream);
}

int mcq_rnorms_from_norms(const float *norms, long B, float *rnorms_out, void *stream) {
    if (B < 0) return MCQ_EINVAL;
    if (B > 0x7fffffffL) return MCQ_EUNSUPPORTED;
    if (B == 0) return 0;
    if (!norms || !rnorms_out) return MCQ_EINVAL;
    hipLaunchKernelGGL(k_rnorms_from_norms, dim3((unsigned)((B + 255) / 256)), dim3(256), 0, static_cast<hipStream_t>(stream),
                       norms, B, rnorms_out);
    return launch_rc();
}

int mcq_search_scan(const float *tables, long Q, const uint8_t *codes, const float *norms, long B, int N, int K, int k,
                    float *out_score, int64_t *out_index, void *workspace, size_t workspace_bytes, void *stream) {
    return mcq_search_scan_metric(tables, Q, codes, norms, B, N, K, k, MCQ_SEARCH_L2, out_score, out_index, workspace,
                                  workspace_bytes, stream);
}

int mcq_search_scan_metric(const float *tables, long Q, const uint8_t *codes, const float *w, long B, int N, int K, int k,
                           int metric, float *out_score, int64_t *out_index, void *workspace, size_t workspace_bytes,
                           void *stream) {
    if (const int rc = search_check(tables, Q, codes, w, B, N, K, k, metric, Q == 0 || (out_score && out_index), workspace))
        return rc;
    if (Q == 0) return 0;
    hipStream_t st = static_cast<hipStream_t>(stream);
    ScanPlan p{};
    float *ws_s = nullptr;
    int *ws_i = nullptr;
    if (B > 0) {
        p = scan_plan(Q, B, N, K, k);
        if (workspace_bytes < 2 * p.ws_half) return MCQ_EWORKSPACE;
        ws_s = static_cast<float *>(workspace);
        ws_i = reinterpret_cast<int *>(static_cast<char *>(workspace) + p.ws_half);
        int rc = MCQ_EUNSUPPORTED;
        switch (metric) {
            case MCQ_SEARCH_L2: rc = launch_scan_qt<kMetricL2>(p, st, tables, (int)Q, codes, w, B, N, K, k, ws_s, ws_i); break;
            case MCQ_SEARCH_IP: rc = launch_scan_qt<kMetricIP>(p, st, tables, (int)Q, codes, nullptr, B, N, K, k, ws_s, ws_i); break;
            case MCQ_SEARCH_COS: rc = launch_scan_qt<kMetricCos>(p, st, tables, (int)Q, codes, w, B, N, K, k, ws_s, ws_i); break;
        }
        if (rc != 0) return rc;
    }
    hipLaunchKernelGGL(k_search_merge, dim3((unsigned)Q), dim3(64), 0, st, ws_s, ws_i, p.slices, k, out_score, out_index);
    return launch_rc();
}

size_t mcq_search_range_workspace_bytes(long Q, long B, int N, int K) {
    if (Q <= 0 || B <= 0 || B > 0x7fffffffL || Q > 0x7fffffffL || search_domain(N, K, 1) != 0) return 256;
    return range_plan(Q, B, N, K).ws_bytes;
}

int mcq_search_range_count(const float *tables, long Q, const uint8_t *codes, const float *w, long B, int N, int K, int metric,
                           const float *thr, int64_t *lims, void *workspace, size_t workspace_bytes, void *stream) {
    if (const int rc = range_check(tables, Q, codes, w, B, N, K, metric, thr, lims, workspace, workspace_bytes)) return rc;
    hipStream_t st = static_cast<hipStream_t>(stream);
    const bool empty = Q == 0 || B == 0;
    if (!empty) {
        const RangePlan p = range_plan(Q, B, N, K);
        int64_t *ws = static_cast<int64_t *>(workspace);
        const RangeArgs a{tables, (int)Q, codes, metric == MCQ_SEARCH_IP ? nullptr : w, B, N, K, metric, thr, ws, nullptr,
                          nullptr, nullptr, 0};
        if (const int rc = launch_range_qt<false>(p, st, a)) return rc;
        hipLaunchKernelGGL(k_range_offsets, dim3((unsigned)Q), dim3(64), 0, st, ws, p.slices * kRangeWaves, lims);
        if (const int rc = launch_rc()) return rc;
    }
    hipLaunchKernelGGL(k_range_lims, dim3(1), dim3(64), 0, st, lims, Q, empty ? 1 : 0);
    return launch_rc();
}

int mcq_search_range_fill(const float *tables, long Q, const uint8_t *codes, const float *w, long B, int N, int K, int metric,
                          const float *thr, const int64_t *lims, float *out_score, int64_t *out_index, long capacity,
                          void *workspace, size_t workspace_bytes, void *stream) {
    if (const int rc = range_check(tables, Q, codes, w, B, N, K, metric, thr, lims, workspace, workspace_bytes)) return rc;
    if (capacity < 0) return MCQ_EINVAL;
    if (Q == 0 || B == 0 || capacity == 0) return 0;
    if (!out_score || !out_index) return MCQ_EINVAL;
    const RangePlan p = range_plan(Q, B, N, K);
    const RangeArgs a{tables, (int)Q, codes, metric == MCQ_SEARCH_IP ? nullptr : w, B, N, K, metric, thr,
                      static_cast<int64_t *>(workspace), lims, out_score, out_index, capacity};
    return launch_range_qt<true>(p, static_cast<hipStream_t>(stream), a);
}

int mcq_last_encode_launches(void) { return g_last_launches; }

int mcq_test_select(const float *scores, int cases, int per_lane, int cnt, float *out_v, int *out_p, void *stream) {
    if (!scores || !out_v || !out_p || cases <= 0 || cnt < 1 || cnt > 64) return MCQ_EINVAL;
    hipStream_t st = static_cast<hipStream_t>(stream);
    switch (per_lane) {
        case 1: hipLaunchKernelGGL((k_test_select<1>), dim3(cases), dim3(64), 0, st, scores, cnt, out_v, out_p); break;
        case 4: hipLaunchKernelGGL((k_test_select<4>), dim3(cases), dim3(64), 0, st, scores, cnt, out_v, out_p); break;
        case 16: hipLaunchKernelGGL((k_test_select<16>), dim3(cases), dim3(64), 0, st, scores, cnt, out_v, out_p); break;
        case -4: hipLaunchKernelGGL((k_test_select<4, kSlotMajor>), dim3(cases), dim3(64), 0, st, scores, cnt, out_v, out_p); break;
        case -16: hipLaunchKernelGGL((k_test_select<16, kSlotMajor>), dim3(cases), dim3(64), 0, st, scores, cnt, out_v, out_p); break;
        case -1004: hipLaunchKernelGGL((k_test_select<4, kAnyOrder>), dim3(cases), dim3(64), 0, st, scores, cnt, out_v, out_p); break;
        default: return MCQ_EINVAL;
    }
    hipError_t e = hipGetLastError();
    return e == hipSuccess ? 0 : (int)e;
}

#ifdef MCQ_STAMPS
int mcq_debug_stamps(unsigned long long *host_dst, long count, int clear) {
    const long total = (long)kStampKernels * kStampWaves * kStampSlots;
    if (count > total) count = total;
    if (hipDeviceSynchronize() != hipSuccess) return MCQ_EINVAL;
    if (host_dst && count > 0 &&
        hipMemcpyFromSymbol(host_dst, HIP_SYMBOL(g_stamps), (size_t)count * 8, 0, hipMemcpyDeviceToHost) != hipSuccess) return MCQ_EINVAL;
    if (clear) {
        void *p = nullptr;
        if (hipGetSymbolAddress(&p, HIP_SYMBOL(g_stamps)) != hipSuccess || hipMemset(p, 0, (size_t)total * 8) != hipSuccess) return MCQ_EINVAL;
    }
    return (int)kStampSlots;
}
#endif

const char *mcq_profile_category_name(int category) {
    return (category >= 0 && category < CAT_COUNT) ? kCatNames[category] : nullptr;
}

int mcq_profile_encode(const float *x, long B, const void *prepared, float lscale_exp, int N, int K, int D,
                       int refine_iters, void *workspace, size_t workspace_bytes, void *stream, float *ms_out,
                       int *launches_out, int cap) {
    hipStream_t st = static_cast<hipStream_t>(stream);
    const bool wide = K > 256;
    const size_t need = (size_t)B * N * (wide ? 8 : 1);
    uint8_t *dummy = nullptr;
    if (!ms_out || cap <= 0) return MCQ_EINVAL;
    const hipError_t me = hipMalloc(reinterpret_cast<void **>(&dummy), need ? need : 1);
    if (me != hipSuccess) return (int)me;
    for (int i = 0; i < cap; ++i) { ms_out[i] = 0.f; if (launches_out) launches_out[i] = 0; }
    int rc = 0;
    for (int only = 0; only < CAT_COUNT && rc == 0; ++only) {
        Prof prof;
        prof.stream = st;
        prof.only = only;
        rc = run_encode(x, B, prepared, lscale_exp, N, K, D, refine_iters, wide ? nullptr : dummy,
                        wide ? reinterpret_cast<int64_t *>(dummy) : nullptr, workspace, workspace_bytes, st, &prof, nullptr,
                        MCQ_ENCODE_ALL_PASSES);
        (void)hipStreamSynchronize(st);
        for (size_t i = 0; rc == 0 && i < prof.cat.size(); ++i) {
            float ms = 0.f;
            (void)hipEventElapsedTime(&ms, prof.ev[prof.first[i]], prof.ev[prof.last[i]]);
            if (prof.cat[i] < cap) { ms_out[prof.cat[i]] += ms; if (launches_out) launches_out[prof.cat[i]] += 1; }
        }
        for (hipEvent_t e : prof.ev) (void)hipEventDestroy(e);
    }
    (void)hipFree(dummy);
    return rc == 0 ? CAT_COUNT : rc;
}

}
```

quantization_amd/csrc/mcq_tf_kernels.h:

```cpp
#pragma once
#include "mcq_kernels.h"

#include <type_traits>

namespace mcq {

constexpr int kTfLevels = 6;

template <int K>
using tf_code_of = std::conditional_t<(K > 256), uint16_t, uint8_t>;

struct TfLists {
    uint8_t *ent;
    uint8_t *pos[kTfLevels];
    float *S[kTfLevels];
    int kc[kTfLevels];
    int64_t *out_i64;
    uint8_t *out_u8;
    int out_pack;
    const int *map;
    const float *erG, *erXC, *erxx;
    float *erE, *erR;
    int erK;
};

__device__ __forceinline__ float shfl_f(float v, int src) {
    return __int_as_float(__builtin_amdgcn_ds_bpermute(src << 2, __float_as_int(v)));
}

#ifdef MCQ_STAMPS
constexpr int kStampSlots = 8, kStampWaves = 1 << 14, kStampKernels = 4;
__device__ unsigned long long g_stamps[kStampKernels * kStampWaves * kStampSlots];
struct Stamps {
    unsigned long long t[kStampSlots];
    __device__ __forceinline__ Stamps() { for (int i = 0; i < kStampSlots; ++i) t[i] = 0; t[0] = __builtin_amdgcn_s_memtime(); }
    __device__ __forceinline__ void at(int k) { asm volatile("s_waitcnt vmcnt(0) lgkmcnt(0)" ::: "memory"); t[k] = __builtin_amdgcn_s_memtime(); }
    __device__ __forceinline__ void flush(int kernel, unsigned wg, int every) {
        if (wg % (unsigned)every != 0 || (threadIdx.x & 63) != 0 || (threadIdx.x >> 6) != 0) return;
        const unsigned slot = (wg / (unsigned)every) & (kStampWaves - 1);
        unsigned long long *d = g_stamps + ((size_t)kernel * kStampWaves + slot) * kStampSlots;
        t[kStampSlots - 1] = __builtin_amdgcn_s_memtime();
        for (int i = 0; i < kStampSlots; ++i) d[i] = t[i];
    }
};
#else
struct Stamps {
    __device__ __forceinline__ void at(int) {}
    __device__ __forceinline__ void flush(int, unsigned, int) {}
};
#endif


template <int N, typename CT = uint8_t>
__global__ void __launch_bounds__(256)
k_tf_gram_terms(const float *__restrict__ G, const CT *__restrict__ idx, long B, int K, float *__restrict__ gterms,
                const int *__restrict__ nact) {
    constexpr int VW = 64 / N;
    if (nact) B = *nact;
    const int m = (int)(blockIdx.x % N);
    const long b = ((long)(blockIdx.x / N) * 4 + (threadIdx.x >> 6)) * VW + lane_id() / N;
    const int m2 = lane_id() % N;
    if (b >= B) return;
    const CT *id = idx + b * N;
    const int NK = N * K;
    gterms[(b * N + m) * N + m2] = G[((size_t)(m * K + id[m]) << __builtin_ctz((unsigned)NK)) + m2 * K + id[m2]];
}

template <int N, bool FROM_REG, typename CT = uint8_t>
__device__ __forceinline__ void tf_er_wave(long b, long bx, const CT *__restrict__ id, int e_reg,
                                           const float *__restrict__ gterms, const float *__restrict__ Gdirect,
                                           const float *__restrict__ XC, const float *__restrict__ xx, int K,
                                           float *__restrict__ E_out, float *__restrict__ R_out) {
    constexpr int NT = (N * N + 63) / 64;
    const int lane = lane_id();
    const int NK = N * K;
#define MCQ_ER_CODE(m) (FROM_REG ? __builtin_amdgcn_ds_bpermute((m) << 2, e_reg) : (int)id[FROM_REG ? 0 : (m)])
    float gt[NT];
#pragma unroll
    for (int j = 0; j < NT; ++j) {
        const int t = lane + 64 * j;
        const int tc = t < N * N ? t : 0;
        const float g = Gdirect ? Gdirect[(size_t)((tc / N) * K + MCQ_ER_CODE(tc / N)) * NK + (tc % N) * K + MCQ_ER_CODE(tc % N)]
                                : gterms[b * (N * N) + tc];
        gt[j] = t < N * N ? g : 0.f;
    }
    const int lm = lane < N ? lane : 0;
    const int clm = MCQ_ER_CODE(lm);
#undef MCQ_ER_CODE
    const float xt = lane < N ? XC[(size_t)bx * NK + lm * K + clm] : 0.f;
    const float xxb = xx[bx];
    float gp = gt[0];
#pragma unroll
    for (int j = 1; j < NT; ++j) gp = gp + gt[j];
    const float gsum = wave_sum_butterfly(gp), xsum = wave_sum_butterfly(xt);
    const float E = (gsum - 2.0f * xsum) + xxb;
    const int n = lane < N ? lane : 0;
    float col = 0.f, gnn = 0.f;
#pragma unroll
    for (int m = 0; m < N; ++m) {
        const float v = shfl_f(gt[(m * N) / 64], (m * N + n) & 63);
        col = (m == 0) ? v : col + v;
        if (m == n) gnn = v;
    }
    const float xo = col - xt;
    const float Rv = (E - 2.0f * xo) + gnn;
    if (lane < N) R_out[b * N + lane] = Rv;
    if (lane == 0) E_out[b] = E;
}

template <int N, typename CT = uint8_t>
__global__ void __launch_bounds__(256)
k_tf_er(const float *__restrict__ gterms, const float *__restrict__ XC, const CT *__restrict__ idx,
        const float *__restrict__ xx, long B, int K, float *__restrict__ E_out, float *__restrict__ R_out,
        const int *__restrict__ nact, const int *__restrict__ map, const float *__restrict__ Gdirect) {
    if (nact) B = *nact;
    const long b = (long)blockIdx.x * 4 + (threadIdx.x >> 6);
    if (b >= B) return;
    const long bx = map ? (long)map[b] : b;
    tf_er_wave<N, false, CT>(b, bx, idx + b * N, 0, gterms, Gdirect, XC, xx, K, E_out, R_out);
}

template <int K, int N>
__device__ __forceinline__ void
tf_stage0_body(unsigned bid, unsigned vgrid, const float *__restrict__ G, const float *__restrict__ XC, const tf_code_of<K> *__restrict__ idx,
               const float *__restrict__ R, const float *__restrict__ Q, long B, int keep,
               tf_code_of<K> *__restrict__ ent_out, float *__restrict__ S_out, tf_code_of<K> *__restrict__ idx_final ,
               const int *__restrict__ nact, const int *__restrict__ map) {
    using CT = tf_code_of<K>;
    constexpr int CB = (int)sizeof(CT);
    constexpr int VPL = (K >= 64) ? K / 64 : 1;
    constexpr int NK = N * K;
    constexpr int CH = (N - 1 < 8) ? (N > 1 ? N - 1 : 1) : 8;
    __shared__ u64 sel[4][kSelectLdsU64];
    Stamps stp;
    if (nact) B = *nact;
    int n;
    long b;
    if constexpr (N > 8) {
        const unsigned per_phase = vgrid / (N / 8);
        const unsigned ph = bid / per_phase, r = bid - ph * per_phase;
        n = (int)(r & 7u) + 8 * (int)ph;
        b = (long)(r >> 3) * 4 + (threadIdx.x >> 6);
    } else {
        n = bid & (N - 1);
        b = (long)(bid / N) * 4 + (threadIdx.x >> 6);
    }
    if (b >= B) return;
    const int lane = lane_id();
    const bool act = VPL * lane < K;
    const int k0 = act ? VPL * lane : 0;
    const CT *id = idx + b * N;
    const float *xc = XC + ((size_t)(map ? (long)map[b] : b) * NK + n * K + k0);
    const float *q = Q + n * K + k0;
    float xcv[VPL], qv[VPL];
    if constexpr (VPL == 4) {
        const f32x4 x4 = __builtin_nontemporal_load(reinterpret_cast<const f32x4 *>(xc)), q4 = *reinterpret_cast<const f32x4 *>(q);
#pragma unroll
        for (int i = 0; i < 4; ++i) { xcv[i] = x4[i]; qv[i] = q4[i]; }
    } else if constexpr (VPL % 4 == 0) {
#pragma unroll
        for (int i4 = 0; i4 < VPL / 4; ++i4) {
            const f32x4 x4 = reinterpret_cast<const f32x4 *>(xc)[i4], q4 = reinterpret_cast<const f32x4 *>(q)[i4];
#pragma unroll
            for (int i = 0; i < 4; ++i) { xcv[4 * i4 + i] = x4[i]; qv[4 * i4 + i] = q4[i]; }
        }
    } else {
#pragma unroll
        for (int i = 0; i < VPL; ++i) { xcv[i] = xc[i]; qv[i] = q[i]; }
    }
    const float Rv = R[(long)__builtin_amdgcn_readfirstlane((int)b) * N + n];
    __builtin_amdgcn_sched_barrier(0);
    unsigned long long iw[N * CB >= 8 ? N * CB / 8 : 1];
    if constexpr (N * CB >= 8) {
        const unsigned long long *ip =
            reinterpret_cast<const unsigned long long *>(idx) + (size_t)__builtin_amdgcn_readfirstlane((int)b) * (N * CB / 8);
#pragma unroll
        for (int q8 = 0; q8 < N * CB / 8; ++q8) iw[q8] = ip[q8];
    }
    auto code = [&](int m) -> int {
        if constexpr (N * CB >= 8) return (int)((iw[(m * CB) >> 3] >> (8 * ((m * CB) & 7))) & (CB == 1 ? 0xffull : 0xffffull));
        else return (int)id[m];
    };
    float t[VPL];
#pragma unroll
    for (int i = 0; i < VPL; ++i) t[i] = 0.f;
#pragma unroll
    for (int j0 = 0; j0 < N - 1; j0 += CH) {
        float gv[CH][VPL];
#pragma unroll
        for (int u = 0; u < CH; ++u) {
            const int j = j0 + u < N - 1 ? j0 + u : N - 2;
            const int m = j < n ? j : j + 1;
            const float *p = G + ((size_t)(m * K + code(m)) * NK + n * K + k0);
            if constexpr (VPL % 4 == 0) {
#pragma unroll
                for (int i4 = 0; i4 < VPL / 4; ++i4) {
                    const f32x4 t4 = reinterpret_cast<const f32x4 *>(p)[i4];
#pragma unroll
                    for (int i = 0; i < 4; ++i) gv[u][4 * i4 + i] = t4[i];
                }
            } else {
#pragma unroll
                for (int i = 0; i < VPL; ++i) gv[u][i] = p[i];
            }
        }
#pragma unroll
        for (int u = 0; u < CH; ++u)
            if (j0 + u < N - 1) {
#pragma unroll
                for (int i = 0; i < VPL; ++i) t[i] = (j0 + u == 0) ? gv[u][i] : t[i] + gv[u][i];
            }
    }
    float sv[VPL];
    int sp[VPL];
#pragma unroll
    for (int i = 0; i < VPL; ++i) {
        const float X = t[i] - xcv[i];
        sv[i] = act ? (Rv + qv[i]) + 2.0f * X : INFINITY;
        sp[i] = act ? k0 + i : kBigPos;
    }
    stp.at(1);
    float ov;
    int op, dst;
    bool has;
    wave_select_set<VPL>(sv, sp, keep, K, sel[threadIdx.x >> 6], has, dst, ov, op);
    stp.at(2);
    stp.flush(0, bid, 16);
    if (N == 1) {
        if (lane == 0) idx_final[b] = (CT)op;
        return;
    }
    if (has) {
        ent_out[(b * N + n) * keep + dst] = (CT)op;
        S_out[(b * N + n) * keep + dst] = ov;
    }
}

template <int K, int N, bool STRIDED = false>
__global__ void __launch_bounds__(256)
k_tf_stage0(const float *__restrict__ G, const float *__restrict__ XC, const tf_code_of<K> *__restrict__ idx,
            const float *__restrict__ R, const float *__restrict__ Q, long B, int keep,
            tf_code_of<K> *__restrict__ ent_out, float *__restrict__ S_out, tf_code_of<K> *__restrict__ idx_final ,
            const int *__restrict__ nact, const int *__restrict__ map, unsigned vgrid) {
    if constexpr (!STRIDED) {
        tf_stage0_body<K, N>(blockIdx.x, gridDim.x, G, XC, idx, R, Q, B, keep, ent_out, S_out, idx_final, nact, map);
        return;
    }
    const unsigned per = (N > 8) ? vgrid / (N / 8) : vgrid;
    const unsigned nr = nact ? (unsigned)((*nact + 3) / 4) * (N > 8 ? 8u : (unsigned)N) : per;
    const unsigned need = (N > 8) ? nr * (N / 8) : nr;
    for (unsigned c = blockIdx.x; c < need; c += gridDim.x) {
        const unsigned vb = (N > 8) ? (c / nr) * per + c % nr : c;
        tf_stage0_body<K, N>(vb, vgrid, G, XC, idx, R, Q, B, keep, ent_out, S_out, idx_final, nact, map);
        wave_lds_fence();
    }
}

template <int N>
__global__ void __launch_bounds__(256)
k_tf_stage0_k16(const float *__restrict__ G, const float *__restrict__ XC, const uint8_t *__restrict__ idx,
                const float *__restrict__ R, const float *__restrict__ Q, long B, int keep,
                uint8_t *__restrict__ ent_out, float *__restrict__ S_out, const int *__restrict__ nact,
                const int *__restrict__ map) {
    static_assert(N >= 4, "");
    constexpr int K = 16, NK = N * K, NG = N / 4;
    if (nact) B = *nact;
    const long w = (long)blockIdx.x * 4 + (threadIdx.x >> 6);
    const long b = w / NG;
    const int n0 = 4 * (int)(w % NG);
    if (b >= B) return;
    const int lane = lane_id();
    const int n = n0 + (lane >> 4), k = lane & 15;
    const float xcv = XC[(size_t)(map ? (long)map[b] : b) * NK + n0 * K + lane];
    const float qv = Q[n0 * K + lane];
    const float Rv = R[b * N + n];
    const long bu = __builtin_amdgcn_readfirstlane((int)b);
    unsigned long long iw[N >= 8 ? N / 8 : 1];
    if constexpr (N >= 8) {
        const unsigned long long *ip = reinterpret_cast<const unsigned long long *>(idx) + (size_t)bu * (N / 8);
#pragma unroll
        for (int q8 = 0; q8 < N / 8; ++q8) iw[q8] = ip[q8];
    } else {
        iw[0] = (unsigned long long)reinterpret_cast<const uint32_t *>(idx)[bu];
    }
    auto code = [&](int m) -> int { return (int)((iw[m >> 3] >> (8 * (m & 7))) & 0xffull) & (K - 1); };
    constexpr int CH = N < 8 ? N : 8;
    float t = 0.f;
    bool started = false;
#pragma unroll
    for (int m0 = 0; m0 < N; m0 += CH) {
        float gv[CH];
#pragma unroll
        for (int u = 0; u < CH; ++u) gv[u] = G[(size_t)((m0 + u) * K + code(m0 + u)) * NK + n0 * K + lane];
#pragma unroll
        for (int u = 0; u < CH; ++u) {
            const bool use = (m0 + u) != n;
            const float sum = t + gv[u];
            t = use ? (started ? sum : gv[u]) : t;
            started = started || use;
        }
    }
    const float X = t - xcv;
    const float sv = (Rv + qv) + 2.0f * X;
    const uint32_t hi = ord32(sv), lo = (uint32_t)k;
    const u64 key = ((u64)hi << 32) | lo;
    int rnk = 0;
#define MCQ_ROR(r)                                                                                                      \
    {                                                                                                                   \
        const u64 o = ((u64)(uint32_t)dpp_i<0x120 + r>((int)hi) << 32) | (uint32_t)dpp_i<0x120 + r>((int)lo);           \
        rnk += (o < key) ? 1 : 0;                                                                                       \
    }
    MCQ_ROR(1) MCQ_ROR(2) MCQ_ROR(3) MCQ_ROR(4) MCQ_ROR(5) MCQ_ROR(6) MCQ_ROR(7) MCQ_ROR(8)
    MCQ_ROR(9) MCQ_ROR(10) MCQ_ROR(11) MCQ_ROR(12) MCQ_ROR(13) MCQ_ROR(14) MCQ_ROR(15)
#undef MCQ_ROR
    const bool take = rnk < keep;
    const u64 tm = __ballot(take);
    const uint32_t rowbits = (uint32_t)(tm >> (lane & 48)) & 0xffffu;
    const int dst = __popc(rowbits & ((1u << k) - 1u));
    if (take) {
        ent_out[(b * N + n) * keep + dst] = (uint8_t)k;
        S_out[(b * N + n) * keep + dst] = sv;
    }
}

template <int KC, typename CT = uint8_t>
__device__ __forceinline__ void tf_leaf(const float *__restrict__ G, int NK, int K, int n, int m,
                                        const CT *__restrict__ en, const CT *__restrict__ em, int old_n,
                                        int old_m, float (&d)[KC * KC / 64]) {
    constexpr int VPL = KC * KC / 64;
    const int lane = lane_id();
    const int i = (VPL * lane) / KC, j0 = (VPL * lane) % KC;
    const uint32_t rown = (uint32_t)(n * K), colm = (uint32_t)(m * K);
    const int nksh = __builtin_ctz((unsigned)NK);
    const int bl = lane < 2 * KC ? lane : 2 * KC;
    const CT *bp = bl < KC ? en + bl : em + (bl < 2 * KC ? bl - KC : 0);
    int e_i = en[i], e_b = *bp;
    uint32_t w4 = 0;
    int ej[VPL];
    constexpr bool kPacked = (VPL == 4 && sizeof(CT) == 1);
    if constexpr (kPacked) {
        w4 = *reinterpret_cast<const uint32_t *>(em + j0);
        asm volatile("" : "+v"(e_i), "+v"(e_b), "+v"(w4));
    } else {
#pragma unroll
        for (int v = 0; v < VPL; ++v) ej[v] = em[j0 + v];
        asm volatile("" : "+v"(e_i), "+v"(e_b), "+v"(ej[0]));
    }
    const uint32_t si = rown + (uint32_t)e_i;
    const uint32_t br = bl < KC ? rown + (uint32_t)e_b : rown + (uint32_t)old_n;
    const uint32_t bc = (bl >= KC && bl < 2 * KC) ? colm + (uint32_t)e_b : colm + (uint32_t)old_m;
    float g[VPL];
    if constexpr (kPacked) {
#pragma unroll
        for (int v = 0; v < 4; ++v) g[v] = G[(si << nksh) + colm + ((w4 >> (8 * v)) & 0xffu)];
    } else {
#pragma unroll
        for (int v = 0; v < VPL; ++v) g[v] = G[(si << nksh) + colm + (uint32_t)ej[v]];
    }
    const float bv = G[(br << nksh) + bc];
    const float u = shfl_f(bv, i), w = shfl_f(bv, 2 * KC);
#pragma unroll
    for (int v = 0; v < VPL; ++v) {
        const float vj = shfl_f(bv, KC + j0 + v);
        d[v] = ((g[v] - u) - vj) + w;
    }
}

__device__ __attribute__((noinline)) void tf_er_next(const float *G, const float *XC, const float *xx, int K, float *E, float *R,
                                                     long b, long bx, int N, int e) {
    if (N == 8) tf_er_wave<8, true, uint8_t>(b, bx, nullptr, e, nullptr, G, XC, xx, K, E, R);
    else if (N == 4) tf_er_wave<4, true, uint8_t>(b, bx, nullptr, e, nullptr, G, XC, xx, K, E, R);
    else if (N == 16) tf_er_wave<16, true, uint8_t>(b, bx, nullptr, e, nullptr, G, XC, xx, K, E, R);
}

template <typename CT>
__device__ __forceinline__ void tf_emit(const TfLists &L, long b, int N, int nlev, int win, CT *__restrict__ idx_out) {
    const int n = lane_id();
    int e = 0;
    if (n < N) {
        int v = nlev - 1;
        int g = n >> v;
        int p = (g & 1) ? win % L.kc[v] : win / L.kc[v];
        while (v > 0) {
            const int child = (n >> (v - 1)) & 1;
            p = L.pos[v][((b * (N >> v) + g) * L.kc[v] + p) * 2 + child];
            --v;
            g = n >> v;
        }
        e = reinterpret_cast<const CT *>(L.ent)[(b * N + n) * L.kc[0] + p];
        idx_out[b * N + n] = (CT)e;
    }
    const long row = (L.map && (L.out_i64 || L.out_u8 || L.erE)) ? (long)L.map[b] : b;
    if (L.out_i64 && n < N) L.out_i64[row * N + n] = e;
    if (L.out_u8) {
        if (L.out_pack == 2) {
            const int hi = __builtin_amdgcn_ds_bpermute(((n + 1) & 63) << 2, e);
            if (n < N && (n & 1) == 0) L.out_u8[row * (N / 2) + n / 2] = (uint8_t)(e + 16 * hi);
        } else if (n < N) {
            L.out_u8[row * N + n] = (uint8_t)e;
        }
    }
    if (L.erE) tf_er_next(L.erG, L.erXC, L.erxx, L.erK, L.erE, L.erR, b, row, N, e);
}

template <int VPL, typename CT = uint8_t, int LAYOUT = kLaneMajor>
__device__ __forceinline__ void tf_finish(const float (&sv)[VPL], const int (&sp)[VPL], int keep, int KCin, u64 *scratch,
                                          const TfLists &L, int vout , long b, int N,
                                          int gout, CT *__restrict__ idx_final) {
    if (idx_final != nullptr) {
        float bv = INFINITY;
        int bp = kBigPos;
#pragma unroll
        for (int i = 0; i < VPL; ++i) lexmin(bv, bp, sv[i], sp[i]);
        wave_lexmin(bv, bp);
        int win = __builtin_amdgcn_readfirstlane(bp);
        if (win > KCin * KCin - 1) win = KCin * KCin - 1;
        tf_emit(L, b, N, vout, win, idx_final);
        return;
    }
    float ov;
    int op, dst;
    bool has;
    wave_select_set<VPL, LAYOUT>(sv, sp, keep, KCin * KCin, scratch, has, dst, ov, op);
    if (has) {
        const long o = (b * (N >> vout) + gout) * keep + dst;
        L.pos[vout][2 * o] = (uint8_t)(op / KCin);
        L.pos[vout][2 * o + 1] = (uint8_t)(op % KCin);
        L.S[vout][o] = ov;
    }
}

template <int KC, typename CT = uint8_t>
__global__ void __launch_bounds__(64)
k_tf_pair0(const float *__restrict__ G, const CT *__restrict__ idx, const float *__restrict__ E, TfLists L, long B,
           int N, int K, int keep, CT *__restrict__ idx_final, const int *__restrict__ nact) {
    constexpr int VPL = KC * KC / 64;
    __shared__ u64 scratch[kSelectLdsU64];
    Stamps stp;
    if (nact) B = *nact;
    const int Gout = N >> 1;
    const int g = (int)(blockIdx.x & (unsigned)(Gout - 1));
    const long b = (long)(blockIdx.x >> __builtin_ctz((unsigned)Gout));
    if (b >= B) return;
    const int lane = lane_id();
    const int n = 2 * g, m = n + 1;
    const CT *en = reinterpret_cast<const CT *>(L.ent) + (b * N + n) * KC, *em = reinterpret_cast<const CT *>(L.ent) + (b * N + m) * KC;
    const int i = (VPL * lane) / KC, j0 = (VPL * lane) % KC;
    const float Eb = E[b];
    const float se = L.S[0][(b * N + n) * KC + i];
    float so[VPL];
#pragma unroll
    for (int v = 0; v < VPL; ++v) so[v] = L.S[0][(b * N + m) * KC + j0 + v];
    float d[VPL];
    stp.at(1);
    tf_leaf<KC, CT>(G, N * K, K, n, m, en, em, idx[b * N + n], idx[b * N + m], d);
    float sv[VPL];
    int sp[VPL];
#pragma unroll
    for (int v = 0; v < VPL; ++v) {
        sv[v] = ((se + so[v]) - Eb) + 2.0f * d[v];
        sp[v] = VPL * lane + v;
    }
    stp.at(2);
    tf_finish<VPL, CT>(sv, sp, keep, KC, scratch, L, 1, b, N, g, idx_final);
    stp.at(3);
    stp.flush(1, blockIdx.x, 64);
}

__device__ __forceinline__ void
tf_pair0s_body(unsigned bid, const float *__restrict__ G, const uint8_t *__restrict__ idx, const float *__restrict__ E, const TfLists &L,
               long B, int N, int K, int keep, uint8_t *__restrict__ idx_final, const int *__restrict__ nact) {
    constexpr int KC = 16, VPL = 4;
    __shared__ u64 scratch[kSelectLdsU64];
    Stamps stp;
    if (nact) B = *nact;
    const int Gout = N >> 1;
    const int g = (int)(bid & (unsigned)(Gout - 1));
    const long b = (long)(bid >> __builtin_ctz((unsigned)Gout));
    if (b >= B) return;
    const int lane = lane_id();
    const int n = 2 * g, m = n + 1;
    const int q4 = lane >> 4, c = lane & 15;
    const uint8_t *en = L.ent + (b * N + n) * KC, *em = en + KC;
    const float *Sn = L.S[0] + (b * N + n) * KC, *Sm = Sn + KC;
    const uint32_t *enw = reinterpret_cast<const uint32_t *>(en);
    uint32_t rw[VPL];
#pragma unroll
    for (int v = 0; v < VPL; ++v) rw[v] = enw[v];
    int e_j = em[c];
    int e_b = en[c];
    int old_n = idx[b * N + n], old_m = idx[b * N + m];
    const float sn_c = Sn[c], so = Sm[c];
    const float Eb = E[b];
    asm volatile("" : "+v"(e_j), "+v"(e_b), "+v"(old_n), "+v"(old_m));
    stp.at(1);
    const int nksh = __builtin_ctz((unsigned)(N * K));
    const uint32_t rown = (uint32_t)(n * K), colm = (uint32_t)(m * K);
    float gq[VPL];
#pragma unroll
    for (int v = 0; v < VPL; ++v) {
        const uint32_t e_i = (rw[v] >> (8 * q4)) & 0xffu;
        gq[v] = G[((rown + e_i) << nksh) + colm + (uint32_t)e_j];
    }
    const uint32_t br = lane < KC ? rown + (uint32_t)e_b : rown + (uint32_t)old_n;
    const uint32_t bc = (lane >= KC && lane < 2 * KC) ? colm + (uint32_t)e_j : colm + (uint32_t)old_m;
    const float bv = G[(br << nksh) + bc];
    const float vj = shfl_f(bv, KC + c), w = shfl_f(bv, 2 * KC);
    float sv[VPL];
    int sp[VPL];
#pragma unroll
    for (int v = 0; v < VPL; ++v) {
        const int i = 4 * v + q4;
        const float u = shfl_f(bv, i), se = shfl_f(sn_c, i);
        const float d = ((gq[v] - u) - vj) + w;
        sv[v] = ((se + so) - Eb) + 2.0f * d;
        sp[v] = 64 * v + lane;
    }
    stp.at(2);
    tf_finish<VPL, uint8_t, kSlotMajor>(sv, sp, keep, KC, scratch, L, 1, b, N, g, idx_final);
    stp.at(3);
    stp.flush(1, bid, 64);
}

template <bool STRIDED = false>
__global__ void __launch_bounds__(64)
k_tf_pair0s(const float *__restrict__ G, const uint8_t *__restrict__ idx, const float *__restrict__ E, TfLists L, long B,
            int N, int K, int keep, uint8_t *__restrict__ idx_final, const int *__restrict__ nact) {
    if constexpr (!STRIDED) {
        tf_pair0s_body(blockIdx.x, G, idx, E, L, B, N, K, keep, idx_final, nact);
        return;
    }
    const unsigned need = nact ? (unsigned)*nact * (unsigned)(N >> 1) : gridDim.x;
    for (unsigned c = blockIdx.x; c < need; c += gridDim.x) {
        tf_pair0s_body(c, G, idx, E, L, B, N, K, keep, idx_final, nact);
        wave_lds_fence();
    }
}

template <int KCH, int KC, typename CT = uint8_t>
__device__ __forceinline__ void tf_table1(const float *__restrict__ G, const CT *__restrict__ idx, const TfLists &L,
                                          long b, int N, int K, int X, int Y, float *leaf ,
                                          float (&t)[KC * KC / 64], Stamps &stp) {
    constexpr int VPLH = KCH * KCH / 64, VPL = KC * KC / 64, MH = KCH * KCH;
    const int lane = lane_id();
    const CT *id = idx + b * N;
    const CT *ent = reinterpret_cast<const CT *>(L.ent);
    const int G1 = N >> 1;
    const uint8_t *px = L.pos[1] + ((b * G1 + X) * KC) * 2, *py = L.pos[1] + ((b * G1 + Y) * KC) * 2;
    if constexpr (KCH == 16 && KC == 16) {
        constexpr int RS = KCH + 1, BO = KCH * RS;
        constexpr int LS = BO + 36;
        CT *cent = reinterpret_cast<CT *>(leaf + 4 * LS);
        uint8_t *crank = reinterpret_cast<uint8_t *>(cent + 64);
        const int NK = N * K;
        const int nksh = __builtin_ctz((unsigned)NK);
        const int w = lane >> 4, c = lane & 15;
        const int cb = (w < 2) ? 2 * X + w : 2 * Y + (w - 2);
        int mypos = (w < 2 ? px : py)[2 * c + (w & 1)];
        int myent = ent[(b * N + cb) * KCH + c];
        int oldv = id[cb];
        asm volatile("" : "+v"(mypos), "+v"(myent), "+v"(oldv));
        stp.at(1);
        int oldq[4];
#pragma unroll
        for (int qq = 0; qq < 4; ++qq) oldq[qq] = __builtin_amdgcn_readlane(oldv, 16 * qq);
        uint32_t m = 1u << mypos;
        m |= (uint32_t)dpp_i<0x121>((int)m);
        m |= (uint32_t)dpp_i<0x122>((int)m);
        m |= (uint32_t)dpp_i<0x124>((int)m);
        m |= (uint32_t)dpp_i<0x128>((int)m);
        crank[lane] = (uint8_t)__popc(m & ((1u << mypos) - 1u));
        if ((m >> c) & 1u) cent[w * 16 + __popc(m & ((1u << c) - 1u))] = (CT)myent;
        uint32_t mq[4];
        mq[0] = (uint32_t)__builtin_amdgcn_readlane((int)m, 0);
        mq[1] = (uint32_t)__builtin_amdgcn_readlane((int)m, 16);
        mq[2] = (uint32_t)__builtin_amdgcn_readlane((int)m, 32);
        mq[3] = (uint32_t)__builtin_amdgcn_readlane((int)m, 48);
        wave_lds_fence();
        int na_[4], nc_[4];
        uint32_t rown_[4], colm_[4];
        float bv[4];
#pragma unroll
        for (int tb = 0; tb < 4; ++tb) {
            const int a = tb >> 1, cc = tb & 1;
            const int n = 2 * X + a, mcb = 2 * Y + cc;
            na_[tb] = __popc(mq[a]);
            nc_[tb] = __popc(mq[2 + cc]);
            rown_[tb] = (uint32_t)(n * K);
            colm_[tb] = (uint32_t)(mcb * K);
            const bool isu = lane < na_[tb], isv = lane >= na_[tb] && lane < na_[tb] + nc_[tb];
            const uint32_t br = rown_[tb] + (uint32_t)(isu ? cent[a * 16 + lane] : oldq[a]);
            const uint32_t bc = colm_[tb] + (uint32_t)(isv ? cent[(2 + cc) * 16 + (lane - na_[tb])] : oldq[2 + cc]);
            bv[tb] = G[isu ? (bc << nksh) + br : (br << nksh) + bc];
        }
        float g[4][4];
        int rr[4][4];
#pragma unroll
        for (int tb = 0; tb < 4; ++tb) {
            const int a = tb >> 1, cc = tb & 1;
            const int na = na_[tb], nc = nc_[tb];
            const float rnc = 1.0f / (float)nc;
#pragma unroll
            for (int it = 0; it < 4; ++it) {
                const int q = lane + 64 * it;
                rr[tb][it] = -1;
                g[tb][it] = 0.f;
                if (64 * it < na * nc) {
                    const int qc = q < na * nc ? q : 0;
                    int ra = (int)((float)qc * rnc);
                    ra -= (ra * nc > qc);
                    ra += ((ra + 1) * nc <= qc);
                    const int rc = qc - ra * nc;
                    g[tb][it] = G[((rown_[tb] + (uint32_t)cent[a * 16 + ra]) << nksh) + colm_[tb] + (uint32_t)cent[(2 + cc) * 16 + rc]];
                    rr[tb][it] = q < na * nc ? ra * 16 + rc : -1;
                }
            }
        }
        stp.at(2);
#pragma unroll
        for (int tb = 0; tb < 4; ++tb)
            if (lane <= na_[tb] + nc_[tb]) leaf[tb * LS + BO + lane] = bv[tb];
        wave_lds_fence();
#pragma unroll
        for (int tb = 0; tb < 4; ++tb) {
            float *lt = leaf + tb * LS;
            const float wv = lt[BO + na_[tb] + nc_[tb]];
#pragma unroll
            for (int it = 0; it < 4; ++it) {
                const int e = rr[tb][it];
                if (e >= 0) lt[e + (e >> 4)] = ((g[tb][it] - lt[BO + (e >> 4)]) - lt[BO + na_[tb] + (e & 15)]) + wv;
            }
        }
        wave_lds_fence();
        const int i = lane >> 2, j0 = 4 * (lane & 3);
        const int ri0 = crank[i], ri1 = crank[16 + i];
#pragma unroll
        for (int v = 0; v < VPL; ++v) {
            const int rj0 = crank[32 + j0 + v], rj1 = crank[48 + j0 + v];
            t[v] = ((leaf[ri0 * RS + rj0] + leaf[LS + ri0 * RS + rj1]) + leaf[2 * LS + ri1 * RS + rj0]) +
                   leaf[3 * LS + ri1 * RS + rj1];
        }
        stp.at(3);
        return;
    } else if constexpr (KCH * KCH == 64) {
        const int NK = N * K;
        const int nksh = __builtin_ctz((unsigned)NK);
        const int i = lane / KCH, j = lane % KCH;
        const int bl = lane < 2 * KCH ? lane : 2 * KCH;
        int cbk[4] = {2 * X, 2 * X + 1, 2 * Y, 2 * Y + 1};
        int e_row[2], e_col[2], e_brd[4], oldq[4];
#pragma unroll
        for (int a = 0; a < 2; ++a) {
            e_row[a] = ent[(b * N + cbk[a]) * KCH + i];
            e_col[a] = ent[(b * N + cbk[2 + a]) * KCH + j];
        }
#pragma unroll
        for (int q4 = 0; q4 < 4; ++q4) {
            oldq[q4] = id[cbk[q4]];
            e_brd[q4] = ent[(b * N + cbk[q4]) * KCH + (q4 < 2 ? (bl < KCH ? bl : 0) : (bl >= KCH && bl < 2 * KCH ? bl - KCH : 0))];
        }
        asm volatile("" : "+v"(e_row[0]), "+v"(e_row[1]), "+v"(e_col[0]), "+v"(e_col[1]));
        asm volatile("" : "+v"(e_brd[0]), "+v"(e_brd[1]), "+v"(e_brd[2]), "+v"(e_brd[3]));
        float g[4], bv[4];
#pragma unroll
        for (int a = 0; a < 2; ++a)
#pragma unroll
            for (int c = 0; c < 2; ++c) {
                const uint32_t rown = (uint32_t)(cbk[a] * K), colm = (uint32_t)(cbk[2 + c] * K);
                g[a * 2 + c] = G[((rown + (uint32_t)e_row[a]) << nksh) + colm + (uint32_t)e_col[c]];
                const uint32_t br = bl < KCH ? rown + (uint32_t)e_brd[a] : rown + (uint32_t)oldq[a];
                const uint32_t bc = (bl >= KCH && bl < 2 * KCH) ? colm + (uint32_t)e_brd[2 + c] : colm + (uint32_t)oldq[2 + c];
                bv[a * 2 + c] = G[(br << nksh) + bc];
            }
        constexpr int RS = KCH + 1, TS = KCH * RS;
#pragma unroll
        for (int tb = 0; tb < 4; ++tb) {
            const float u = shfl_f(bv[tb], i), w = shfl_f(bv[tb], 2 * KCH), vj = shfl_f(bv[tb], KCH + j);
            leaf[tb * TS + i * RS + j] = ((g[tb] - u) - vj) + w;
        }
        wave_lds_fence();
        const int ii = (VPL * lane) / KC, j0 = (VPL * lane) % KC;
        const int i0 = px[2 * ii], i1 = px[2 * ii + 1];
#pragma unroll
        for (int v = 0; v < VPL; ++v) {
            const int jj0 = py[2 * (j0 + v)], jj1 = py[2 * (j0 + v) + 1];
            t[v] = ((leaf[i0 * RS + jj0] + leaf[TS + i0 * RS + jj1]) + leaf[2 * TS + i1 * RS + jj0]) +
                   leaf[3 * TS + i1 * RS + jj1];
        }
    } else {
#pragma unroll
        for (int a = 0; a < 2; ++a)
#pragma unroll
            for (int c = 0; c < 2; ++c) {
                const int n = 2 * X + a, m = 2 * Y + c;
                float d[VPLH];
                tf_leaf<KCH, CT>(G, N * K, K, n, m, ent + (b * N + n) * KCH, ent + (b * N + m) * KCH, id[n], id[m], d);
                float *dst = leaf + (a * 2 + c) * MH + VPLH * lane;
#pragma unroll
                for (int v = 0; v < VPLH; ++v) dst[v] = d[v];
            }
        wave_lds_fence();
        const int i = (VPL * lane) / KC, j0 = (VPL * lane) % KC;
        const int i0 = px[2 * i], i1 = px[2 * i + 1];
#pragma unroll
        for (int v = 0; v < VPL; ++v) {
            const int jj0 = py[2 * (j0 + v)], jj1 = py[2 * (j0 + v) + 1];
            t[v] = ((leaf[i0 * KCH + jj0] + leaf[MH + i0 * KCH + jj1]) + leaf[2 * MH + i1 * KCH + jj0]) +
                   leaf[3 * MH + i1 * KCH + jj1];
        }
    }
}


constexpr int tf_leaf_lds_floats(int KCH, int code_bytes = 1) { return 4 * (KCH * (KCH + 1) + 36) + 16 + 16 * code_bytes; }

template <int KCH, int KC, typename CT = uint8_t>
__device__ __forceinline__ void tf_pair1_body(unsigned bid, float *leaf, const float *__restrict__ G, const CT *__restrict__ idx,
                                              const float *__restrict__ E, const TfLists &L, long B, int N, int K, int keep,
                                              CT *__restrict__ idx_final, const int *__restrict__ nact) {
    constexpr int VPL = KC * KC / 64;
    static_assert(tf_leaf_lds_floats(KCH, sizeof(CT)) * 4 >= kSelectLdsU64 * 8, "");
    u64 *scratch = reinterpret_cast<u64 *>(leaf);
    Stamps stp;
    if (nact) B = *nact;
    const int Gout = N >> 2;
    const int g = (int)(bid & (unsigned)(Gout - 1));
    const long b = (long)(bid >> __builtin_ctz((unsigned)Gout));
    if (b >= B) return;
    const int lane = lane_id();
    const int X = 2 * g, Y = X + 1, G1 = N >> 1;
    const int i = (VPL * lane) / KC, j0 = (VPL * lane) % KC;
    const float Eb = E[b];
    const float se = L.S[1][(b * G1 + X) * KC + i];
    float so[VPL];
#pragma unroll
    for (int v = 0; v < VPL; ++v) so[v] = L.S[1][(b * G1 + Y) * KC + j0 + v];
    float t[VPL];
    tf_table1<KCH, KC, CT>(G, idx, L, b, N, K, X, Y, leaf, t, stp);
    float sv[VPL];
    int sp[VPL];
#pragma unroll
    for (int v = 0; v < VPL; ++v) {
        sv[v] = ((se + so[v]) - Eb) + 2.0f * t[v];
        sp[v] = VPL * lane + v;
    }
    wave_lds_fence();
    tf_finish<VPL, CT>(sv, sp, keep, KC, scratch, L, 2, b, N, g, idx_final);
    stp.at(4);
    stp.flush(2, bid, 64);
}

template <int KCH, int KC, typename CT = uint8_t>
__global__ void __launch_bounds__(64)
k_tf_pair1(const float *__restrict__ G, const CT *__restrict__ idx, const float *__restrict__ E, TfLists L, long B,
           int N, int K, int keep, CT *__restrict__ idx_final, const int *__restrict__ nact) {
    __shared__ __attribute__((aligned(16))) float leaf[tf_leaf_lds_floats(KCH, sizeof(CT))];
    tf_pair1_body<KCH, KC, CT>(blockIdx.x, leaf, G, idx, E, L, B, N, K, keep, idx_final, nact);
}

template <int KCH, int KC, typename CT = uint8_t>
__device__ __forceinline__ void tf_table1_body(unsigned bid, float *leaf, const float *__restrict__ G, const CT *__restrict__ idx,
                                               const TfLists &L, long B, int N, int K, int ntab, int per, float *__restrict__ tabs,
                                               const int *__restrict__ nact) {
    constexpr int VPL = KC * KC / 64;
    Stamps stp;
    if (nact) B = *nact;
    const int t = (int)(bid & (unsigned)(ntab - 1));
    const long b = (long)(bid >> __builtin_ctz((unsigned)ntab));
    if (b >= B) return;
    const int lane = lane_id();
    const int psh = __builtin_ctz((unsigned)per);
    const int c = t & (per - 1), a = (t >> psh) & (per - 1), g = t >> (2 * psh);
    const int X = 2 * g * per + a, Y = (2 * g + 1) * per + c;
    float tv[VPL];
    tf_table1<KCH, KC, CT>(G, idx, L, b, N, K, X, Y, leaf, tv, stp);
    float *dst = tabs + ((size_t)(b * ntab + t) * (KC * KC) + VPL * lane);
    if constexpr (VPL == 4) {
        __builtin_nontemporal_store((f32x4){tv[0], tv[1], tv[2], tv[3]}, reinterpret_cast<f32x4 *>(dst));
    } else {
#pragma unroll
        for (int v = 0; v < VPL; ++v) dst[v] = tv[v];
    }
    stp.at(4);
    stp.flush(3, bid, 64);
}

template <int KCH, int KC, typename CT = uint8_t>
__global__ void __launch_bounds__(64)
k_tf_table1(const float *__restrict__ G, const CT *__restrict__ idx, TfLists L, long B, int N, int K, int ntab,
            int per, float *__restrict__ tabs, const int *__restrict__ nact) {
    __shared__ __attribute__((aligned(16))) float leaf[tf_leaf_lds_floats(KCH, sizeof(CT))];
    tf_table1_body<KCH, KC, CT>(blockIdx.x, leaf, G, idx, L, B, N, K, ntab, per, tabs, nact);
}

template <int KCH, int KC, typename CT = uint8_t, bool STRIDED = false>
__global__ void __launch_bounds__(64)
k_tf_level1(const float *__restrict__ G, const CT *__restrict__ idx, const float *__restrict__ E, TfLists L, long B, int N,
            int K, int keep, int ntab, int per, float *__restrict__ tabs, const int *__restrict__ nact, unsigned pair_blocks,
            unsigned tab_blocks, int ntab2, int per2, float *__restrict__ tabs2, unsigned vgrid) {
    __shared__ __attribute__((aligned(16))) float leaf[tf_leaf_lds_floats(KCH, sizeof(CT))];
    if constexpr (!STRIDED) {
        if (blockIdx.x < pair_blocks) tf_pair1_body<KCH, KC, CT>(blockIdx.x, leaf, G, idx, E, L, B, N, K, keep, nullptr, nact);
        else if (blockIdx.x < pair_blocks + tab_blocks) tf_table1_body<KCH, KC, CT>(blockIdx.x - pair_blocks, leaf, G, idx, L, B, N, K, ntab, per, tabs, nact);
        else tf_table1_body<KCH, KC, CT>(blockIdx.x - pair_blocks - tab_blocks, leaf, G, idx, L, B, N, K, ntab2, per2, tabs2, nact);
        return;
    }
    unsigned r0 = pair_blocks, r1 = tab_blocks, r2 = vgrid - pair_blocks - tab_blocks;
    if (nact) {
        const unsigned na = (unsigned)*nact;
        r0 = (na * (unsigned)(N / 4) + 7u) & ~7u;
        r1 = (na * (unsigned)ntab + 7u) & ~7u;
        r2 = r2 ? na * (unsigned)ntab2 : 0u;
    }
    for (unsigned c = blockIdx.x; c < r0 + r1 + r2; c += gridDim.x) {
        if (c < r0) tf_pair1_body<KCH, KC, CT>(c, leaf, G, idx, E, L, B, N, K, keep, nullptr, nact);
        else if (c < r0 + r1) tf_table1_body<KCH, KC, CT>(c - r0, leaf, G, idx, L, B, N, K, ntab, per, tabs, nact);
        else tf_table1_body<KCH, KC, CT>(c - r0 - r1, leaf, G, idx, L, B, N, K, ntab2, per2, tabs2, nact);
        wave_lds_fence();
    }
}

template <int KH>
constexpr int tf_tab_stride() { return KH * (KH + 1); }

template <int KH, int COUNT>
__device__ __forceinline__ void tf_load_tables(const float *__restrict__ src, float *dst) {
    constexpr int M = KH * KH, RS = KH + 1, TS = tf_tab_stride<KH>();
    const int lane = lane_id();
    if constexpr ((COUNT * M) % 256 == 0 && KH % 4 == 0) {
        constexpr int IT = COUNT * M / 256;
        constexpr int BATCH = IT < 8 ? IT : 8;
#pragma unroll
        for (int i0 = 0; i0 < IT; i0 += BATCH) {
            f32x4 r[BATCH];
#pragma unroll
            for (int i = 0; i < BATCH; ++i)
                if (i0 + i < IT) r[i] = __builtin_nontemporal_load(reinterpret_cast<const f32x4 *>(src) + lane + 64 * (i0 + i));
#pragma unroll
            for (int i = 0; i < BATCH; ++i)
                if (i0 + i < IT) {
                    const int e = 4 * (lane + 64 * (i0 + i));
                    float *d = dst + (e / M) * TS + ((e % M) / KH) * RS + (e % KH);
#pragma unroll
                    for (int c = 0; c < 4; ++c) d[c] = r[i][c];
                }
        }
    } else {
        constexpr int TOT = COUNT * M;
        constexpr int IT = (TOT + 63) / 64;
        float r[IT];
#pragma unroll
        for (int i = 0; i < IT; ++i) r[i] = (lane + 64 * i < TOT) ? src[lane + 64 * i] : 0.f;
#pragma unroll
        for (int i = 0; i < IT; ++i) {
            const int e = lane + 64 * i;
            if (e < TOT) dst[(e / M) * TS + ((e % M) / KH) * RS + (e % KH)] = r[i];
        }
    }
}

template <int KH, int KC>
__device__ __forceinline__ void tf_up(const float *t00, const float *t01, const float *t10, const float *t11,
                                      const uint8_t *__restrict__ px, const uint8_t *__restrict__ py,
                                      float (&t)[KC * KC / 64]) {
    constexpr int VPL = KC * KC / 64;
    const int lane = lane_id();
    const int i = (VPL * lane) / KC, j0 = (VPL * lane) % KC;
    const int i0 = px[2 * i], i1 = px[2 * i + 1];
#pragma unroll
    for (int v = 0; v < VPL; ++v) {
        const int jj0 = py[2 * (j0 + v)], jj1 = py[2 * (j0 + v) + 1];
        t[v] = ((t00[i0 * (KH + 1) + jj0] + t01[i0 * (KH + 1) + jj1]) + t10[i1 * (KH + 1) + jj0]) + t11[i1 * (KH + 1) + jj1];
    }
}

template <int KH, int KC>
__global__ void __launch_bounds__(64)
k_tf_up(TfLists L, long B, int N, int u, int ntab, int per, const float *__restrict__ tabs_in, float *__restrict__ tabs_out,
        const int *__restrict__ nact) {
    constexpr int VPL = KC * KC / 64, MH = KH * KH, TS = tf_tab_stride<KH>();
    __shared__ __attribute__((aligned(16))) float th[4 * TS];
    if (nact) B = *nact;
    const int t = (int)(blockIdx.x & (unsigned)(ntab - 1));
    const long b = (long)(blockIdx.x >> __builtin_ctz((unsigned)ntab));
    if (b >= B) return;
    const int lane = lane_id();
    const int psh = __builtin_ctz((unsigned)per);
    const int c = t & (per - 1), a = (t >> psh) & (per - 1), g = t >> (2 * psh);
    const int X = 2 * g * per + a, Y = (2 * g + 1) * per + c;
    const int Gu = N >> u;
    const size_t cbase = (size_t)b * (4 * ntab) + (size_t)g * (4 * per * per);
#pragma unroll
    for (int i = 0; i < 2; ++i)
#pragma unroll
        for (int j = 0; j < 2; ++j)
            tf_load_tables<KH, 1>(tabs_in + (cbase + (size_t)(2 * a + i) * (2 * per) + (2 * c + j)) * MH, th + (2 * i + j) * TS);
    wave_lds_fence();
    float tv[VPL];
    tf_up<KH, KC>(th, th + TS, th + 2 * TS, th + 3 * TS, L.pos[u] + ((b * Gu + X) * KC) * 2, L.pos[u] + ((b * Gu + Y) * KC) * 2, tv);
    float *dst = tabs_out + ((size_t)(b * ntab + t) * (KC * KC) + VPL * lane);
#pragma unroll
    for (int v = 0; v < VPL; ++v) __builtin_nontemporal_store(tv[v], dst + v);
}

template <int KH, int KC, bool LAST, typename CT = uint8_t>
__device__ __forceinline__ void
tf_comb_body(unsigned bid, const float *__restrict__ E, const TfLists &L, long B, int N, int v, int keep, const float *__restrict__ tabs,
             CT *__restrict__ idx_final, const int *__restrict__ nact) {
    constexpr int MH = KH * KH, RS = KH + 1, TS = tf_tab_stride<KH>();
    constexpr int VPL = (KC * KC / 64 <= 16) ? KC * KC / 64 : 16;
    constexpr int CHUNKS = KC * KC / (64 * VPL);
    constexpr int LDSF = (4 * TS * 4 >= kSelectLdsU64 * 8) ? 4 * TS : kSelectLdsU64 * 2;
    __shared__ __attribute__((aligned(16))) float th[LDSF];
    u64 *scratch = reinterpret_cast<u64 *>(th);
    __shared__ u64 sel2_store[(KC * KC / 64 > 16) ? kSelectLdsU64 : 1];
    u64 *sel2 = sel2_store;
    if (nact) B = *nact;
    const int Gout = N >> (v + 1);
    const int h = (int)(bid & (unsigned)(Gout - 1));
    const long b = (long)(bid >> __builtin_ctz((unsigned)Gout));
    if (b >= B) return;
    const int lane = lane_id();
    const int P = 2 * h, Q = P + 1, Gv = N >> v;
    tf_load_tables<KH, 4>(tabs + ((size_t)b * Gout + h) * 4 * MH, th);
    const float Eb = E[b];
    const uint8_t *px = L.pos[v] + ((b * Gv + P) * KC) * 2, *py = L.pos[v] + ((b * Gv + Q) * KC) * 2;
    const float *Sx = L.S[v] + (b * Gv + P) * KC, *Sy = L.S[v] + (b * Gv + Q) * KC;
    wave_lds_fence();
    if constexpr (CHUNKS == 1 && !LAST) {
        const int i = (VPL * lane) / KC, j0 = (VPL * lane) % KC;
        const float se = Sx[i];
        float t[VPL];
        tf_up<KH, KC>(th, th + TS, th + 2 * TS, th + 3 * TS, px, py, t);
        float sv[VPL];
        int sp[VPL];
#pragma unroll
        for (int u = 0; u < VPL; ++u) {
            sv[u] = ((se + Sy[j0 + u]) - Eb) + 2.0f * t[u];
            sp[u] = VPL * lane + u;
        }
        wave_lds_fence();
        tf_finish<VPL, CT>(sv, sp, keep, KC, scratch, L, v + 1, b, N, h, idx_final);
    } else if (!LAST) {
        static_assert(CHUNKS <= 4, "");
        float cv[4];
        int cp[4];
#pragma unroll
        for (int c = 0; c < 4; ++c) { cv[c] = INFINITY; cp[c] = kBigPos; }
        for (int c = 0; c < CHUNKS; ++c) {
            const int p0 = 64 * VPL * c + VPL * lane;
            const int i = p0 / KC, j0 = p0 % KC;
            const int i0 = px[2 * i], i1 = px[2 * i + 1];
            const float se = Sx[i];
            float sv[VPL];
            int sp[VPL];
#pragma unroll
            for (int u = 0; u < VPL; ++u) {
                const int jj0 = py[2 * (j0 + u)], jj1 = py[2 * (j0 + u) + 1];
                const float t = ((th[i0 * RS + jj0] + th[TS + i0 * RS + jj1]) + th[2 * TS + i1 * RS + jj0]) + th[3 * TS + i1 * RS + jj1];
                sv[u] = ((se + Sy[j0 + u]) - Eb) + 2.0f * t;
                sp[u] = p0 + u;
            }
            float ov;
            int op, dst;
            bool got;
            wave_select_set<VPL>(sv, sp, keep, KC * KC, sel2, got, dst, ov, op);
#pragma unroll
            for (int q = 0; q < 4; ++q)
                if (q == c) { cv[q] = got ? ov : INFINITY; cp[q] = got ? op : kBigPos; }
        }
        tf_finish<4, CT, kAnyOrder>(cv, cp, keep, KC, sel2, L, v + 1, b, N, h, nullptr);
    } else {
        float bv = INFINITY;
        int bp = kBigPos;
        for (int c = 0; c < CHUNKS; ++c) {
            const int p0 = 64 * VPL * c + VPL * lane;
            const int i = p0 / KC, j0 = p0 % KC;
            const int i0 = px[2 * i], i1 = px[2 * i + 1];
            const float se = Sx[i];
#pragma unroll
            for (int u = 0; u < VPL; ++u) {
                const int jj0 = py[2 * (j0 + u)], jj1 = py[2 * (j0 + u) + 1];
                const float t = ((th[i0 * RS + jj0] + th[TS + i0 * RS + jj1]) + th[2 * TS + i1 * RS + jj0]) + th[3 * TS + i1 * RS + jj1];
                lexmin(bv, bp, ((se + Sy[j0 + u]) - Eb) + 2.0f * t, p0 + u);
            }
        }
        wave_lexmin(bv, bp);
        if (bp > KC * KC - 1) bp = KC * KC - 1;
        tf_emit(L, b, N, v + 1, bp, idx_final);
    }
}

template <int KH, int KC, bool LAST, typename CT = uint8_t, bool STRIDED = false>
__global__ void __launch_bounds__(64)
k_tf_comb(const float *__restrict__ E, TfLists L, long B, int N, int v, int keep, const float *__restrict__ tabs,
          CT *__restrict__ idx_final, const int *__restrict__ nact) {
    if constexpr (!STRIDED) {
        tf_comb_body<KH, KC, LAST, CT>(blockIdx.x, E, L, B, N, v, keep, tabs, idx_final, nact);
        return;
    }
    const unsigned need = nact ? (unsigned)*nact * (unsigned)(N >> (v + 1)) : gridDim.x;
    for (unsigned c = blockIdx.x; c < need; c += gridDim.x) {
        tf_comb_body<KH, KC, LAST, CT>(c, E, L, B, N, v, keep, tabs, idx_final, nact);
        wave_lds_fence();
    }
}

template <int KC1, int KC2, int KC3, typename CT = uint8_t>
__global__ void __launch_bounds__(256)
k_tf_comb3(const CT *__restrict__ idx, const float *__restrict__ E, TfLists L, long B, int N,
           const float *__restrict__ tabs, CT *__restrict__ idx_final, const int *__restrict__ nact) {
    constexpr int VPL2 = KC2 * KC2 / 64, M1 = KC1 * KC1;
    constexpr int PW = KC3 * KC3 / 4, VPLW = PW / 64;
    constexpr int RS1 = KC1 + 1, TS1 = tf_tab_stride<KC1>(), RS2 = KC2 + 1, TS2 = KC2 * RS2;
    __shared__ __attribute__((aligned(16))) float t1[16 * TS1];
    __shared__ __attribute__((aligned(16))) float t2[4 * TS2];
    __shared__ float wv[4];
    __shared__ int wp[4];
    (void)idx;
    if (nact) B = *nact;
    const long b = blockIdx.x;
    if (b >= B) return;
    const int lane = lane_id(), w = threadIdx.x >> 6;
    const int G2 = N >> 2;
    const int xc = w >> 1, yc = w & 1;
    constexpr int NB2 = 2 * VPL2;
    const int i2 = (VPL2 * lane) / KC2, j2 = (VPL2 * lane) % KC2;
    const uint8_t *px2 = L.pos[2] + ((b * G2 + xc) * KC2) * 2, *py2 = L.pos[2] + ((b * G2 + 2 + yc) * KC2) * 2;
    const unsigned pxw2 = *reinterpret_cast<const uint16_t *>(px2 + 2 * i2);
    uint32_t pyw2[NB2 / 4];
#pragma unroll
    for (int u = 0; u < NB2 / 4; ++u) pyw2[u] = reinterpret_cast<const uint32_t *>(py2 + 2 * j2)[u];
    const uint8_t *px = L.pos[3] + ((b * 2 + 0) * KC3) * 2, *py = L.pos[3] + ((b * 2 + 1) * KC3) * 2;
    const float *Sx = L.S[3] + (b * 2 + 0) * KC3, *Sy = L.S[3] + (b * 2 + 1) * KC3;
    const int p0 = w * PW + VPLW * lane;
    const int i3 = p0 / KC3, j3 = p0 % KC3;
    const unsigned pxw3 = *reinterpret_cast<const uint16_t *>(px + 2 * i3);
    unsigned pyw3[VPLW];
    float sy3[VPLW];
#pragma unroll
    for (int v = 0; v < VPLW; ++v) {
        pyw3[v] = *reinterpret_cast<const uint16_t *>(py + 2 * (j3 + v));
        sy3[v] = Sy[j3 + v];
    }
    const float sx3 = Sx[i3];
    const float Eb = E[b];
    tf_load_tables<KC1, 4>(tabs + ((size_t)b * 16 + 4 * w) * M1, t1 + 4 * w * TS1);
    __builtin_amdgcn_sched_barrier(0);
    __syncthreads();
    {
        const int X0 = 2 * xc, Y0 = 2 * yc;
        const float *t00 = t1 + (4 * X0 + Y0) * TS1, *t01 = t1 + (4 * X0 + Y0 + 1) * TS1, *t10 = t1 + (4 * (X0 + 1) + Y0) * TS1,
                    *t11 = t1 + (4 * (X0 + 1) + Y0 + 1) * TS1;
        const int i0 = (int)(pxw2 & 0xffu), i1 = (int)(pxw2 >> 8);
        float *dst = t2 + w * TS2 + i2 * RS2 + j2;
#pragma unroll
        for (int v = 0; v < VPL2; ++v) {
            const uint32_t wj = pyw2[v >> 1] >> (16 * (v & 1));
            const int jj0 = (int)(wj & 0xffu), jj1 = (int)((wj >> 8) & 0xffu);
            dst[v] = ((t00[i0 * RS1 + jj0] + t01[i0 * RS1 + jj1]) + t10[i1 * RS1 + jj0]) + t11[i1 * RS1 + jj1];
        }
    }
    __syncthreads();
    float bv = INFINITY;
    int bp = kBigPos;
    {
        const int i0 = (int)(pxw3 & 0xffu), i1 = (int)(pxw3 >> 8);
#pragma unroll
        for (int v = 0; v < VPLW; ++v) {
            const int jj0 = (int)(pyw3[v] & 0xffu), jj1 = (int)(pyw3[v] >> 8);
            const float t = ((t2[i0 * RS2 + jj0] + t2[TS2 + i0 * RS2 + jj1]) + t2[2 * TS2 + i1 * RS2 + jj0]) + t2[3 * TS2 + i1 * RS2 + jj1];
            lexmin(bv, bp, ((sx3 + sy3[v]) - Eb) + 2.0f * t, p0 + v);
        }
    }
    wave_lexmin(bv, bp);
    if (lane == 0) { wv[w] = bv; wp[w] = bp; }
    __syncthreads();
    if (w == 0) {
        float rv = wv[0];
        int rp = wp[0];
#pragma unroll
        for (int u = 1; u < 4; ++u) lexmin(rv, rp, wv[u], wp[u]);
        if (rp > KC3 * KC3 - 1) rp = KC3 * KC3 - 1;
        tf_emit(L, b, N, 4, rp, idx_final);
    }
}

}
```

Before: 13.87 million vectors/s.

## Precompute cross-codebook border terms in stage0 and reuse them in pair/table kernels

Stage0 now writes a small per-vector 'border' buffer holding the G cross terms between each codebook's kept candidates and the other codebooks' current codes, taken from values it already has in registers. The pair0s, pair1 and table1 kernels read these precomputed borders instead of doing scattered gathers into the large G matrix, which removes dependent index loads and random global reads. In exchange stage0 does extra LDS work and global stores, and a new workspace buffer is added. The buffer reuses tabs[1] when there is room. The path is on by default for K 32-256 and N 2-8, and can be turned off with an environment variable.

```diff
diff --git a/quantization_amd/csrc/mcq_api.hip b/quantization_amd/csrc/mcq_api.hip
--- a/quantization_amd/csrc/mcq_api.hip
+++ b/quantization_amd/csrc/mcq_api.hip
@@ -79,6 +79,7 @@
     int8_t *xf;
     int *xe;
     float *tabs[2];
+    float *brd;
     TfLists tf;
 };
 
@@ -100,10 +101,18 @@
 
 inline size_t code_bytes_of(int K) { return K > 256 ? 2 : 1; }
 
+inline bool tf_borders_enabled() {
+    static const bool on = !(getenv("MCQ_TF_BORDERS") && atoi(getenv("MCQ_TF_BORDERS")) == 0);
+    return on;
+}
+size_t tf_border_bytes(int N, int K) {
+    return (tf_borders_shape(K, N, (int)code_bytes_of(K)) && N != 8) ? (size_t)N * N * kTfBorderW * 4 : 0;
+}
+
 size_t workspace_per_vector(int N, int K, int D) {
     const size_t cb = code_bytes_of(K);
     return 4 * cb * (size_t)N + 8 + 8 + 4 * (size_t)N + 4 * (size_t)N * K + (size_t)tf_levels(N) * N * (16 * cb + 2 * 16 + 4 * 16) + 64 +
-           2 * 4 * tf_tab_floats(N, K) + 4 * (size_t)fix_round_cols(D) + 4 + 4 * (size_t)N * N;
+           2 * 4 * tf_tab_floats(N, K) + 4 * (size_t)fix_round_cols(D) + 4 + 4 * (size_t)N * N + tf_border_bytes(N, K);
 }
 size_t workspace_slack(int D) { return 48 * 256 + (size_t)kFixTile * (4 * (size_t)fix_round_cols(D) + 4); }
 
@@ -154,6 +163,12 @@
     }
     const size_t tf = tf_tab_floats(N, K);
     for (int i = 0; i < 2; ++i) w.tabs[i] = tf ? reinterpret_cast<float *>(take((size_t)Bc * tf * 4)) : nullptr;
+    w.brd = nullptr;
+    if (tf_borders_shape(K, N, (int)sizeof(CT))) {
+        float *room = tf_border_bytes(N, K) ? reinterpret_cast<float *>(take((size_t)Bc * tf_border_bytes(N, K)))
+                                            : (tf >= (size_t)N * N * kTfBorderW ? w.tabs[1] : nullptr);
+        if (tf_borders_enabled()) w.brd = room;
+    }
     return w;
 }
 
@@ -296,13 +311,13 @@
 template <int K>
 int launch_tf_stage0_k(int N, const float *G, const float *XC, const tf_code_of<K> *idx, const float *R, const float *Q, long B,
                        int keep, tf_code_of<K> *ent, float *S, tf_code_of<K> *fin, const int *nact, const int *map, hipStream_t st,
-                       bool capped) {
+                       bool capped, float *brd) {
     const unsigned vgrid = (unsigned)(((B + 3) / 4) * N);
     const dim3 grid(pass_grid(vgrid, capped, kCapStage0)), block(256);
 #define MCQ_S0_CASE(NN)                                                                                                            \
     case NN:                                                                                                                       \
-        if (capped) hipLaunchKernelGGL((k_tf_stage0<K, NN, true>), grid, block, 0, st, G, XC, idx, R, Q, B, keep, ent, S, fin, nact, map, vgrid); \
-        else hipLaunchKernelGGL((k_tf_stage0<K, NN, false>), grid, block, 0, st, G, XC, idx, R, Q, B, keep, ent, S, fin, nact, map, vgrid);      \
+        if (capped) hipLaunchKernelGGL((k_tf_stage0<K, NN, true>), grid, block, 0, st, G, XC, idx, R, Q, B, keep, ent, S, fin, nact, map, vgrid, brd); \
+        else hipLaunchKernelGGL((k_tf_stage0<K, NN, false>), grid, block, 0, st, G, XC, idx, R, Q, B, keep, ent, S, fin, nact, map, vgrid, brd); \
         break;
     switch (N) {
         MCQ_S0_CASE(1) MCQ_S0_CASE(2) MCQ_S0_CASE(4) MCQ_S0_CASE(8) MCQ_S0_CASE(16) MCQ_S0_CASE(32) MCQ_S0_CASE(64)
@@ -315,17 +330,17 @@
 
 int launch_tf_stage0(int K, int N, const float *G, const float *XC, const uint16_t *idx, const float *R, const float *Q,
                      long B, int keep, uint16_t *ent, float *S, uint16_t *fin, const int *nact, const int *map, hipStream_t st,
-                     bool capped) {
+                     bool capped, float *brd) {
     switch (K) {
-        case 512: return launch_tf_stage0_k<512>(N, G, XC, idx, R, Q, B, keep, ent, S, fin, nact, map, st, capped);
-        case 1024: return launch_tf_stage0_k<1024>(N, G, XC, idx, R, Q, B, keep, ent, S, fin, nact, map, st, capped);
+        case 512: return launch_tf_stage0_k<512>(N, G, XC, idx, R, Q, B, keep, ent, S, fin, nact, map, st, capped, brd);
+        case 1024: return launch_tf_stage0_k<1024>(N, G, XC, idx, R, Q, B, keep, ent, S, fin, nact, map, st, capped, brd);
         default: return MCQ_EUNSUPPORTED;
     }
 }
 
 int launch_tf_stage0(int K, int N, const float *G, const float *XC, const uint8_t *idx, const float *R, const float *Q,
                      long B, int keep, uint8_t *ent, float *S, uint8_t *fin, const int *nact, const int *map, hipStream_t st,
-                     bool capped) {
+                     bool capped, float *brd) {
     if (K == 16 && N >= 4 && keep <= 16) {
         const dim3 grid((unsigned)((B * (N / 4) + 3) / 4)), block(256);
 #define MCQ_S16_CASE(NN) \
@@ -339,11 +354,11 @@
         return 0;
     }
     switch (K) {
-        case 16: return launch_tf_stage0_k<16>(N, G, XC, idx, R, Q, B, keep, ent, S, fin, nact, map, st, capped);
-        case 32: return launch_tf_stage0_k<32>(N, G, XC, idx, R, Q, B, keep, ent, S, fin, nact, map, st, capped);
-        case 64: return launch_tf_stage0_k<64>(N, G, XC, idx, R, Q, B, keep, ent, S, fin, nact, map, st, capped);
-        case 128: return launch_tf_stage0_k<128>(N, G, XC, idx, R, Q, B, keep, ent, S, fin, nact, map, st, capped);
-        case 256: return launch_tf_stage0_k<256>(N, G, XC, idx, R, Q, B, keep, ent, S, fin, nact, map, st, capped);
+        case 16: return launch_tf_stage0_k<16>(N, G, XC, idx, R, Q, B, keep, ent, S, fin, nact, map, st, capped, brd);
+        case 32: return launch_tf_stage0_k<32>(N, G, XC, idx, R, Q, B, keep, ent, S, fin, nact, map, st, capped, brd);
+        case 64: return launch_tf_stage0_k<64>(N, G, XC, idx, R, Q, B, keep, ent, S, fin, nact, map, st, capped, brd);
+        case 128: return launch_tf_stage0_k<128>(N, G, XC, idx, R, Q, B, keep, ent, S, fin, nact, map, st, capped, brd);
+        case 256: return launch_tf_stage0_k<256>(N, G, XC, idx, R, Q, B, keep, ent, S, fin, nact, map, st, capped, brd);
         default: return MCQ_EUNSUPPORTED;
     }
 }
@@ -451,9 +466,9 @@
             if (!small) {
                 if (capped)
                     hipLaunchKernelGGL(k_tf_pair0s<true>, dim3(pass_grid(grid.x, true, kCapWave)), dim3(64), 0, st, G, idx_cur, w.E, L, B, N,
-                                       K, keep, fin, nact);
+                                       K, keep, fin, nact, w.brd);
                 else
-                    hipLaunchKernelGGL(k_tf_pair0s<false>, grid, dim3(64), 0, st, G, idx_cur, w.E, L, B, N, K, keep, fin, nact);
+                    hipLaunchKernelGGL(k_tf_pair0s<false>, grid, dim3(64), 0, st, G, idx_cur, w.E, L, B, N, K, keep, fin, nact, w.brd);
                 done0 = true;
             }
         }
@@ -473,10 +488,10 @@
         if (prof) prof->begin(CAT_LEVEL1_FUSED);
         if (capped)
             MCQ_TF_LAUNCH2((k_tf_level1<8, 8, CT, true>), (k_tf_level1<16, 16, CT, true>), grid, dim3(64), G, idx_cur, w.E, L, B, N, K, keep, ntab1,
-                           per1, w.tabs[0], nact, pair_blocks, tab_blocks, ntab3, per3, w.tabs[1], vgrid);
+                           per1, w.tabs[0], nact, pair_blocks, tab_blocks, ntab3, per3, w.tabs[1], vgrid, w.brd);
         else
             MCQ_TF_LAUNCH2((k_tf_level1<8, 8, CT>), (k_tf_level1<16, 16, CT>), grid, dim3(64), G, idx_cur, w.E, L, B, N, K, keep, ntab1, per1, w.tabs[0],
-                           nact, pair_blocks, tab_blocks, ntab3, per3, w.tabs[1], vgrid);
+                           nact, pair_blocks, tab_blocks, ntab3, per3, w.tabs[1], vgrid, w.brd);
         MCQ_LAUNCH_CHECK();
         if (prof) prof->end(CAT_LEVEL1_FUSED);
     } else if (N >= 4) {
@@ -484,7 +499,7 @@
         CT *fin = (N == 4) ? idx_new : nullptr;
         const dim3 grid((unsigned)(B * (N / 4)));
         if (prof) prof->begin(CAT_LEVEL1);
-        MCQ_TF_LAUNCH2((k_tf_pair1<8, 8, CT>), (k_tf_pair1<16, 16, CT>), grid, dim3(64), G, idx_cur, w.E, L, B, N, K, keep, fin, nact);
+        MCQ_TF_LAUNCH2((k_tf_pair1<8, 8, CT>), (k_tf_pair1<16, 16, CT>), grid, dim3(64), G, idx_cur, w.E, L, B, N, K, keep, fin, nact, w.brd);
         MCQ_LAUNCH_CHECK();
         if (prof) prof->end(CAT_LEVEL1);
     }
@@ -639,7 +654,7 @@
             er_ready = false;
             if (prof) prof->begin(CAT_STAGE0);
             rc = launch_tf_stage0(K, N, P.G, w.XC, idx_cur, R_cur, P.Q, Bc, (N == 1) ? 1 : w.tf.kc[0], reinterpret_cast<CT *>(w.tf.ent),
-                                  w.tf.S[0], (N == 1) ? idx_new : static_cast<CT *>(nullptr), nact, map_cur, st, capped);
+                                  w.tf.S[0], (N == 1) ? idx_new : static_cast<CT *>(nullptr), nact, map_cur, st, capped, w.brd);
             if (rc) return rc;
             if (prof) prof->end(CAT_STAGE0);
             bool direct_out = false;
diff --git a/quantization_amd/csrc/mcq_tf_kernels.h b/quantization_amd/csrc/mcq_tf_kernels.h
--- a/quantization_amd/csrc/mcq_tf_kernels.h
+++ b/quantization_amd/csrc/mcq_tf_kernels.h
@@ -24,6 +24,12 @@
     int erK;
 };
 
+constexpr int kTfBorderW = 16;
+__host__ __device__ constexpr bool tf_borders_shape(int K, int N, int code_bytes) {
+    return code_bytes == 1 && K >= 32 && K <= 256 && N >= 2 && N <= 8;
+}
+typedef float f32x2 __attribute__((ext_vector_type(2)));
+
 __device__ __forceinline__ float shfl_f(float v, int src) {
     return __int_as_float(__builtin_amdgcn_ds_bpermute(src << 2, __float_as_int(v)));
 }
@@ -125,7 +131,7 @@
 tf_stage0_body(unsigned bid, unsigned vgrid, const float *__restrict__ G, const float *__restrict__ XC, const tf_code_of<K> *__restrict__ idx,
                const float *__restrict__ R, const float *__restrict__ Q, long B, int keep,
                tf_code_of<K> *__restrict__ ent_out, float *__restrict__ S_out, tf_code_of<K> *__restrict__ idx_final ,
-               const int *__restrict__ nact, const int *__restrict__ map) {
+               const int *__restrict__ nact, const int *__restrict__ map, float *__restrict__ brd) {
     using CT = tf_code_of<K>;
     constexpr int CB = (int)sizeof(CT);
     constexpr int VPL = (K >= 64) ? K / 64 : 1;
@@ -184,9 +190,9 @@
     float t[VPL];
 #pragma unroll
     for (int i = 0; i < VPL; ++i) t[i] = 0.f;
+    float gv[CH][VPL];
 #pragma unroll
     for (int j0 = 0; j0 < N - 1; j0 += CH) {
-        float gv[CH][VPL];
 #pragma unroll
         for (int u = 0; u < CH; ++u) {
             const int j = j0 + u < N - 1 ? j0 + u : N - 2;
@@ -234,6 +240,38 @@
         ent_out[(b * N + n) * keep + dst] = (CT)op;
         S_out[(b * N + n) * keep + dst] = ov;
     }
+    if constexpr (tf_borders_shape(K, N, CB)) {
+        if (brd != nullptr && keep == kTfBorderW) {
+            uint32_t *lo = reinterpret_cast<uint32_t *>(sel[threadIdx.x >> 6]);
+            uint8_t *rmap = reinterpret_cast<uint8_t *>(lo);
+            float *blk = reinterpret_cast<float *>(lo + 64);
+            if (lane < K / 4) lo[lane] = 0xffffffffu;
+            wave_lds_fence();
+            if (has && (unsigned)op < (unsigned)K) rmap[op] = (uint8_t)dst;
+            wave_lds_fence();
+            const int oc = code(n) - k0;
+#pragma unroll
+            for (int i = 0; i < VPL; ++i) {
+                const int r = act ? (int)rmap[k0 + i] : 0xff;
+                if (r != 0xff) {
+#pragma unroll
+                    for (int u = 0; u < N - 1; ++u) blk[(u < n ? u : u + 1) * kTfBorderW + r] = gv[u][i];
+                }
+                if (act && oc == i) {
+#pragma unroll
+                    for (int u = 0; u < N - 1; ++u) blk[n * kTfBorderW + (u < n ? u : u + 1)] = gv[u][i];
+                }
+            }
+            wave_lds_fence();
+            float *bo = brd + (size_t)(b * N + n) * (N * kTfBorderW);
+            if constexpr (N * kTfBorderW == 128) {
+                __builtin_nontemporal_store(reinterpret_cast<const f32x2 *>(blk)[lane], reinterpret_cast<f32x2 *>(bo) + lane);
+            } else {
+                static_assert(N * kTfBorderW <= 64, "");
+                if (lane < N * kTfBorderW) __builtin_nontemporal_store(blk[lane], bo + lane);
+            }
+        }
+    }
 }
 
 template <int K, int N, bool STRIDED = false>
@@ -241,9 +279,9 @@
 k_tf_stage0(const float *__restrict__ G, const float *__restrict__ XC, const tf_code_of<K> *__restrict__ idx,
             const float *__restrict__ R, const float *__restrict__ Q, long B, int keep,
             tf_code_of<K> *__restrict__ ent_out, float *__restrict__ S_out, tf_code_of<K> *__restrict__ idx_final ,
-            const int *__restrict__ nact, const int *__restrict__ map, unsigned vgrid) {
+            const int *__restrict__ nact, const int *__restrict__ map, unsigned vgrid, float *__restrict__ brd) {
     if constexpr (!STRIDED) {
-        tf_stage0_body<K, N>(blockIdx.x, gridDim.x, G, XC, idx, R, Q, B, keep, ent_out, S_out, idx_final, nact, map);
+        tf_stage0_body<K, N>(blockIdx.x, gridDim.x, G, XC, idx, R, Q, B, keep, ent_out, S_out, idx_final, nact, map, brd);
         return;
     }
     const unsigned per = (N > 8) ? vgrid / (N / 8) : vgrid;
@@ -251,7 +289,7 @@
     const unsigned need = (N > 8) ? nr * (N / 8) : nr;
     for (unsigned c = blockIdx.x; c < need; c += gridDim.x) {
         const unsigned vb = (N > 8) ? (c / nr) * per + c % nr : c;
-        tf_stage0_body<K, N>(vb, vgrid, G, XC, idx, R, Q, B, keep, ent_out, S_out, idx_final, nact, map);
+        tf_stage0_body<K, N>(vb, vgrid, G, XC, idx, R, Q, B, keep, ent_out, S_out, idx_final, nact, map, brd);
         wave_lds_fence();
     }
 }
@@ -469,7 +507,8 @@
 
 __device__ __forceinline__ void
 tf_pair0s_body(unsigned bid, const float *__restrict__ G, const uint8_t *__restrict__ idx, const float *__restrict__ E, const TfLists &L,
-               long B, int N, int K, int keep, uint8_t *__restrict__ idx_final, const int *__restrict__ nact) {
+               long B, int N, int K, int keep, uint8_t *__restrict__ idx_final, const int *__restrict__ nact,
+               const float *__restrict__ brd) {
     constexpr int KC = 16, VPL = 4;
     __shared__ u64 scratch[kSelectLdsU64];
     Stamps stp;
@@ -488,11 +527,21 @@
 #pragma unroll
     for (int v = 0; v < VPL; ++v) rw[v] = enw[v];
     int e_j = em[c];
-    int e_b = en[c];
-    int old_n = idx[b * N + n], old_m = idx[b * N + m];
+    int e_b = 0, old_n = 0, old_m = 0;
+    float bv = 0.f;
+    if (brd != nullptr) {
+        const float *bb = brd + (size_t)b * (N * N * kTfBorderW);
+        if (lane <= 2 * KC)
+            bv = __builtin_nontemporal_load(bb + (lane < KC ? (n * N + m) * kTfBorderW + lane
+                                                 : lane < 2 * KC ? (m * N + n) * kTfBorderW + (lane - KC) : (n * N + n) * kTfBorderW + m));
+    } else {
+        e_b = en[c];
+        old_n = idx[b * N + n];
+        old_m = idx[b * N + m];
+    }
     const float sn_c = Sn[c], so = Sm[c];
     const float Eb = E[b];
-    asm volatile("" : "+v"(e_j), "+v"(e_b), "+v"(old_n), "+v"(old_m));
+    asm volatile("" : "+v"(e_j), "+v"(e_b), "+v"(old_n), "+v"(old_m), "+v"(bv));
     stp.at(1);
     const int nksh = __builtin_ctz((unsigned)(N * K));
     const uint32_t rown = (uint32_t)(n * K), colm = (uint32_t)(m * K);
@@ -502,9 +551,11 @@
         const uint32_t e_i = (rw[v] >> (8 * q4)) & 0xffu;
         gq[v] = G[((rown + e_i) << nksh) + colm + (uint32_t)e_j];
     }
-    const uint32_t br = lane < KC ? rown + (uint32_t)e_b : rown + (uint32_t)old_n;
-    const uint32_t bc = (lane >= KC && lane < 2 * KC) ? colm + (uint32_t)e_j : colm + (uint32_t)old_m;
-    const float bv = G[(br << nksh) + bc];
+    if (brd == nullptr && lane <= 2 * KC) {
+        const uint32_t br = lane < KC ? rown + (uint32_t)e_b : rown + (uint32_t)old_n;
+        const uint32_t bc = (lane >= KC && lane < 2 * KC) ? colm + (uint32_t)e_j : colm + (uint32_t)old_m;
+        bv = G[(br << nksh) + bc];
+    }
     const float vj = shfl_f(bv, KC + c), w = shfl_f(bv, 2 * KC);
     float sv[VPL];
     int sp[VPL];
@@ -525,14 +576,14 @@
 template <bool STRIDED = false>
 __global__ void __launch_bounds__(64)
 k_tf_pair0s(const float *__restrict__ G, const uint8_t *__restrict__ idx, const float *__restrict__ E, TfLists L, long B,
-            int N, int K, int keep, uint8_t *__restrict__ idx_final, const int *__restrict__ nact) {
+            int N, int K, int keep, uint8_t *__restrict__ idx_final, const int *__restrict__ nact, const float *__restrict__ brd) {
     if constexpr (!STRIDED) {
-        tf_pair0s_body(blockIdx.x, G, idx, E, L, B, N, K, keep, idx_final, nact);
+        tf_pair0s_body(blockIdx.x, G, idx, E, L, B, N, K, keep, idx_final, nact, brd);
         return;
     }
     const unsigned need = nact ? (unsigned)*nact * (unsigned)(N >> 1) : gridDim.x;
     for (unsigned c = blockIdx.x; c < need; c += gridDim.x) {
-        tf_pair0s_body(c, G, idx, E, L, B, N, K, keep, idx_final, nact);
+        tf_pair0s_body(c, G, idx, E, L, B, N, K, keep, idx_final, nact, brd);
         wave_lds_fence();
     }
 }
@@ -540,7 +591,7 @@
 template <int KCH, int KC, typename CT = uint8_t>
 __device__ __forceinline__ void tf_table1(const float *__restrict__ G, const CT *__restrict__ idx, const TfLists &L,
                                           long b, int N, int K, int X, int Y, float *leaf ,
-                                          float (&t)[KC * KC / 64], Stamps &stp) {
+                                          float (&t)[KC * KC / 64], Stamps &stp, const float *__restrict__ brd) {
     constexpr int VPLH = KCH * KCH / 64, VPL = KC * KC / 64, MH = KCH * KCH;
     const int lane = lane_id();
     const CT *id = idx + b * N;
@@ -558,8 +609,18 @@
         const int cb = (w < 2) ? 2 * X + w : 2 * Y + (w - 2);
         int mypos = (w < 2 ? px : py)[2 * c + (w & 1)];
         int myent = ent[(b * N + cb) * KCH + c];
-        int oldv = id[cb];
-        asm volatile("" : "+v"(mypos), "+v"(myent), "+v"(oldv));
+        int oldv = 0;
+        float b0 = 0.f, b1 = 0.f, bcn = 0.f;
+        if (brd != nullptr) {
+            const float *bb = brd + (size_t)(b * N + cb) * (N * kTfBorderW);
+            const int oth = (w < 2) ? 2 * Y : 2 * X;
+            b0 = __builtin_nontemporal_load(bb + oth * kTfBorderW + c);
+            b1 = __builtin_nontemporal_load(bb + (oth + 1) * kTfBorderW + c);
+            if (w < 2 && c < 2) bcn = __builtin_nontemporal_load(bb + cb * kTfBorderW + 2 * Y + c);
+        } else {
+            oldv = id[cb];
+        }
+        asm volatile("" : "+v"(mypos), "+v"(myent), "+v"(oldv), "+v"(b0), "+v"(b1), "+v"(bcn));
         stp.at(1);
         int oldq[4];
 #pragma unroll
@@ -588,10 +649,13 @@
             nc_[tb] = __popc(mq[2 + cc]);
             rown_[tb] = (uint32_t)(n * K);
             colm_[tb] = (uint32_t)(mcb * K);
-            const bool isu = lane < na_[tb], isv = lane >= na_[tb] && lane < na_[tb] + nc_[tb];
-            const uint32_t br = rown_[tb] + (uint32_t)(isu ? cent[a * 16 + lane] : oldq[a]);
-            const uint32_t bc = colm_[tb] + (uint32_t)(isv ? cent[(2 + cc) * 16 + (lane - na_[tb])] : oldq[2 + cc]);
-            bv[tb] = G[isu ? (bc << nksh) + br : (br << nksh) + bc];
+            bv[tb] = 0.f;
+            if (brd == nullptr && lane <= na_[tb] + nc_[tb]) {
+                const bool isu = lane < na_[tb], isv = lane >= na_[tb] && lane < na_[tb] + nc_[tb];
+                const uint32_t br = rown_[tb] + (uint32_t)(isu ? cent[a * 16 + lane] : oldq[a]);
+                const uint32_t bc = colm_[tb] + (uint32_t)(isv ? cent[(2 + cc) * 16 + (lane - na_[tb])] : oldq[2 + cc]);
+                bv[tb] = G[isu ? (bc << nksh) + br : (br << nksh) + bc];
+            }
         }
         float g[4][4];
         int rr[4][4];
@@ -605,21 +669,32 @@
                 const int q = lane + 64 * it;
                 rr[tb][it] = -1;
                 g[tb][it] = 0.f;
-                if (64 * it < na * nc) {
-                    const int qc = q < na * nc ? q : 0;
-                    int ra = (int)((float)qc * rnc);
-                    ra -= (ra * nc > qc);
-                    ra += ((ra + 1) * nc <= qc);
-                    const int rc = qc - ra * nc;
+                if (q < na * nc) {
+                    int ra = (int)((float)q * rnc);
+                    ra -= (ra * nc > q);
+                    ra += ((ra + 1) * nc <= q);
+                    const int rc = q - ra * nc;
                     g[tb][it] = G[((rown_[tb] + (uint32_t)cent[a * 16 + ra]) << nksh) + colm_[tb] + (uint32_t)cent[(2 + cc) * 16 + rc]];
-                    rr[tb][it] = q < na * nc ? ra * 16 + rc : -1;
+                    rr[tb][it] = ra * 16 + rc;
                 }
             }
         }
         stp.at(2);
-#pragma unroll
-        for (int tb = 0; tb < 4; ++tb)
-            if (lane <= na_[tb] + nc_[tb]) leaf[tb * LS + BO + lane] = bv[tb];
+        if (brd != nullptr) {
+            const int rk = __popc(m & ((1u << c) - 1u)), nq = __popc(m);
+            const bool inm = (m >> c) & 1u;
+            if (w < 2) {
+                if (inm) { leaf[(2 * w) * LS + BO + rk] = b0; leaf[(2 * w + 1) * LS + BO + rk] = b1; }
+                if (c < 2) leaf[(2 * w + c) * LS + BO + nq + __popc(c == 0 ? mq[2] : mq[3])] = bcn;
+            } else if (inm) {
+                leaf[(w - 2) * LS + BO + __popc(mq[0]) + rk] = b0;
+                leaf[(w) * LS + BO + __popc(mq[1]) + rk] = b1;
+            }
+        } else {
+#pragma unroll
+            for (int tb = 0; tb < 4; ++tb)
+                if (lane <= na_[tb] + nc_[tb]) leaf[tb * LS + BO + lane] = bv[tb];
+        }
         wave_lds_fence();
 #pragma unroll
         for (int tb = 0; tb < 4; ++tb) {
@@ -717,7 +792,8 @@
 template <int KCH, int KC, typename CT = uint8_t>
 __device__ __forceinline__ void tf_pair1_body(unsigned bid, float *leaf, const float *__restrict__ G, const CT *__restrict__ idx,
                                               const float *__restrict__ E, const TfLists &L, long B, int N, int K, int keep,
-                                              CT *__restrict__ idx_final, const int *__restrict__ nact) {
+                                              CT *__restrict__ idx_final, const int *__restrict__ nact,
+                                              const float *__restrict__ brd) {
     constexpr int VPL = KC * KC / 64;
     static_assert(tf_leaf_lds_floats(KCH, sizeof(CT)) * 4 >= kSelectLdsU64 * 8, "");
     u64 *scratch = reinterpret_cast<u64 *>(leaf);
@@ -736,7 +812,7 @@
 #pragma unroll
     for (int v = 0; v < VPL; ++v) so[v] = L.S[1][(b * G1 + Y) * KC + j0 + v];
     float t[VPL];
-    tf_table1<KCH, KC, CT>(G, idx, L, b, N, K, X, Y, leaf, t, stp);
+    tf_table1<KCH, KC, CT>(G, idx, L, b, N, K, X, Y, leaf, t, stp, brd);
     float sv[VPL];
     int sp[VPL];
 #pragma unroll
@@ -753,15 +829,15 @@
 template <int KCH, int KC, typename CT = uint8_t>
 __global__ void __launch_bounds__(64)
 k_tf_pair1(const float *__restrict__ G, const CT *__restrict__ idx, const float *__restrict__ E, TfLists L, long B,
-           int N, int K, int keep, CT *__restrict__ idx_final, const int *__restrict__ nact) {
+           int N, int K, int keep, CT *__restrict__ idx_final, const int *__restrict__ nact, const float *__restrict__ brd) {
     __shared__ __attribute__((aligned(16))) float leaf[tf_leaf_lds_floats(KCH, sizeof(CT))];
-    tf_pair1_body<KCH, KC, CT>(blockIdx.x, leaf, G, idx, E, L, B, N, K, keep, idx_final, nact);
+    tf_pair1_body<KCH, KC, CT>(blockIdx.x, leaf, G, idx, E, L, B, N, K, keep, idx_final, nact, brd);
 }
 
 template <int KCH, int KC, typename CT = uint8_t>
 __device__ __forceinline__ void tf_table1_body(unsigned bid, float *leaf, const float *__restrict__ G, const CT *__restrict__ idx,
                                                const TfLists &L, long B, int N, int K, int ntab, int per, float *__restrict__ tabs,
-                                               const int *__restrict__ nact) {
+                                               const int *__restrict__ nact, const float *__restrict__ brd) {
     constexpr int VPL = KC * KC / 64;
     Stamps stp;
     if (nact) B = *nact;
@@ -773,7 +849,7 @@
     const int c = t & (per - 1), a = (t >> psh) & (per - 1), g = t >> (2 * psh);
     const int X = 2 * g * per + a, Y = (2 * g + 1) * per + c;
     float tv[VPL];
-    tf_table1<KCH, KC, CT>(G, idx, L, b, N, K, X, Y, leaf, tv, stp);
+    tf_table1<KCH, KC, CT>(G, idx, L, b, N, K, X, Y, leaf, tv, stp, brd);
     float *dst = tabs + ((size_t)(b * ntab + t) * (KC * KC) + VPL * lane);
     if constexpr (VPL == 4) {
         __builtin_nontemporal_store((f32x4){tv[0], tv[1], tv[2], tv[3]}, reinterpret_cast<f32x4 *>(dst));
@@ -790,19 +866,19 @@
 k_tf_table1(const float *__restrict__ G, const CT *__restrict__ idx, TfLists L, long B, int N, int K, int ntab,
             int per, float *__restrict__ tabs, const int *__restrict__ nact) {
     __shared__ __attribute__((aligned(16))) float leaf[tf_leaf_lds_floats(KCH, sizeof(CT))];
-    tf_table1_body<KCH, KC, CT>(blockIdx.x, leaf, G, idx, L, B, N, K, ntab, per, tabs, nact);
+    tf_table1_body<KCH, KC, CT>(blockIdx.x, leaf, G, idx, L, B, N, K, ntab, per, tabs, nact, nullptr);
 }
 
 template <int KCH, int KC, typename CT = uint8_t, bool STRIDED = false>
 __global__ void __launch_bounds__(64)
 k_tf_level1(const float *__restrict__ G, const CT *__restrict__ idx, const float *__restrict__ E, TfLists L, long B, int N,
             int K, int keep, int ntab, int per, float *__restrict__ tabs, const int *__restrict__ nact, unsigned pair_blocks,
-            unsigned tab_blocks, int ntab2, int per2, float *__restrict__ tabs2, unsigned vgrid) {
+            unsigned tab_blocks, int ntab2, int per2, float *__restrict__ tabs2, unsigned vgrid, const float *__restrict__ brd) {
     __shared__ __attribute__((aligned(16))) float leaf[tf_leaf_lds_floats(KCH, sizeof(CT))];
     if constexpr (!STRIDED) {
-        if (blockIdx.x < pair_blocks) tf_pair1_body<KCH, KC, CT>(blockIdx.x, leaf, G, idx, E, L, B, N, K, keep, nullptr, nact);
-        else if (blockIdx.x < pair_blocks + tab_blocks) tf_table1_body<KCH, KC, CT>(blockIdx.x - pair_blocks, leaf, G, idx, L, B, N, K, ntab, per, tabs, nact);
-        else tf_table1_body<KCH, KC, CT>(blockIdx.x - pair_blocks - tab_blocks, leaf, G, idx, L, B, N, K, ntab2, per2, tabs2, nact);
+        if (blockIdx.x < pair_blocks) tf_pair1_body<KCH, KC, CT>(blockIdx.x, leaf, G, idx, E, L, B, N, K, keep, nullptr, nact, brd);
+        else if (blockIdx.x < pair_blocks + tab_blocks) tf_table1_body<KCH, KC, CT>(blockIdx.x - pair_blocks, leaf, G, idx, L, B, N, K, ntab, per, tabs, nact, brd);
+        else tf_table1_body<KCH, KC, CT>(blockIdx.x - pair_blocks - tab_blocks, leaf, G, idx, L, B, N, K, ntab2, per2, tabs2, nact, brd);
         return;
     }
     unsigned r0 = pair_blocks, r1 = tab_blocks, r2 = vgrid - pair_blocks - tab_blocks;
@@ -813,9 +889,9 @@
         r2 = r2 ? na * (unsigned)ntab2 : 0u;
     }
     for (unsigned c = blockIdx.x; c < r0 + r1 + r2; c += gridDim.x) {
-        if (c < r0) tf_pair1_body<KCH, KC, CT>(c, leaf, G, idx, E, L, B, N, K, keep, nullptr, nact);
-        else if (c < r0 + r1) tf_table1_body<KCH, KC, CT>(c - r0, leaf, G, idx, L, B, N, K, ntab, per, tabs, nact);
-        else tf_table1_body<KCH, KC, CT>(c - r0 - r1, leaf, G, idx, L, B, N, K, ntab2, per2, tabs2, nact);
+        if (c < r0) tf_pair1_body<KCH, KC, CT>(c, leaf, G, idx, E, L, B, N, K, keep, nullptr, nact, brd);
+        else if (c < r0 + r1) tf_table1_body<KCH, KC, CT>(c - r0, leaf, G, idx, L, B, N, K, ntab, per, tabs, nact, brd);
+        else tf_table1_body<KCH, KC, CT>(c - r0 - r1, leaf, G, idx, L, B, N, K, ntab2, per2, tabs2, nact, brd);
         wave_lds_fence();
     }
 }
```

Measured after the change: 11.98 million vectors/s. -13.6%, worse.
